# aleflabo/MoCoDAD

Hardware: AMD Instinct MI355X
Metric: pose-clips/sec (whole node) @ noise_steps=10, 5 seeds; AUC vs ref (higher is better)
Workload: dtype f32

## Files before the change

### mocodad_amd/csrc/mcd_device.hpp

```cpp

#pragma once
#include <hip/hip_runtime.h>
#include <stdint.h>
#include <string.h>
#include <stdlib.h>
#include <math.h>
#include <string>
#include <vector>
#include <unordered_map>
#include <utility>
#include <type_traits>
#include <atomic>

#include "../../include/mocodad_hip.h"
#include "mcd_chain.hpp"

namespace mcd {

typedef float f32x4 __attribute__((ext_vector_type(4)));
typedef float f32x2 __attribute__((ext_vector_type(2)));
typedef const float __attribute__((address_space(4))) cfloat;
typedef const float __attribute__((address_space(1))) gfloat;
typedef const f32x4 __attribute__((address_space(1))) gf32x4;
__device__ __forceinline__ gfloat* as_global(const float* p) { return (gfloat*)p; }
typedef float __attribute__((address_space(3))) lds_float;
typedef f32x4 __attribute__((address_space(3))) lds_f32x4;
__device__ __forceinline__ unsigned lds_addr(const float* p) { return (unsigned)(uintptr_t)p; }
__device__ __forceinline__ float4 lds_load4(unsigned addr) {
    const f32x4 v = *(lds_f32x4*)(uintptr_t)addr;
    return make_float4(v[0], v[1], v[2], v[3]);
}
__device__ __forceinline__ void lds_store4(unsigned addr, float a, float b, float c, float d) {
    *(lds_f32x4*)(uintptr_t)addr = f32x4{a, b, c, d};
}
typedef f32x4 __attribute__((address_space(1))) gf32x4_rw;
__device__ __forceinline__ void store_global4(float* p, float4 v) {
    *(gf32x4_rw*)p = f32x4{v.x, v.y, v.z, v.w};
}
__device__ __forceinline__ float4 load_global4(const float* p) {
    const f32x4 v = *(gf32x4*)p;
    return make_float4(v[0], v[1], v[2], v[3]);
}

#ifndef MCD_NWAVES
#define MCD_NWAVES 8
#endif
constexpr int NWAVES = MCD_NWAVES;
constexpr int NTHREADS = NWAVES * 64;
constexpr int EDIM = 16;
constexpr int NLAYERS = 11;
constexpr int EMB_TOTAL = 532;
constexpr int EMB_STRIDE = 536;

__host__ __device__ constexpr int cs_of(int c) { return c + 4; }
__host__ __device__ constexpr int ceil16(int x) { return (x + 15) / 16 * 16; }

struct LDesc { int cin, cout, V, res; };
__host__ __device__ constexpr LDesc layer_desc(int l) {
    return l == 0 ? LDesc{16, 16, 17, 1}  : l == 1 ? LDesc{16, 32, 17, 1} : l == 2 ? LDesc{32, 32, 17, 0}
         : l == 3 ? LDesc{32, 64, 12, 1} : l == 4 ? LDesc{64, 64, 12, 0} : l == 5 ? LDesc{64, 128, 10, 1}
         : l == 6 ? LDesc{128, 64, 10, 1} : l == 7 ? LDesc{64, 64, 12, 0} : l == 8 ? LDesc{64, 32, 12, 1}
         : l == 9 ? LDesc{32, 32, 17, 0} : LDesc{32, 2, 17, 1};
}
__host__ __device__ constexpr int emb_off(int l) {
    return l == 0 ? 0 : l == 1 ? 16 : l == 2 ? 48 : l == 3 ? 80 : l == 4 ? 144 : l == 5 ? 208 : l == 6 ? 336
         : l == 7 ? 400 : l == 8 ? 464 : l == 9 ? 496 : 528;
}

constexpr int TAB_FLOATS = 256;
enum { F_TQ = 0, F_AM = 1, F_WP = 2, F_BIAS = 3, F_SLOPE = 4, F_STRIDE = 8 };
constexpr int TAB_WE = 88, TAB_BE = 89;
constexpr int TAB_RSW = 90, TAB_RSB = 94;
typedef const int __attribute__((address_space(4))) cint;
__device__ __forceinline__ int tab_i(const float* base, int idx) { return ((cint*)base)[idx]; }
__device__ __forceinline__ float tab_f(const float* base, int idx) { return ((cfloat*)base)[idx]; }
template <bool U32>
__device__ __forceinline__ const float* wptr(const float* wb, int off) {
    if constexpr (U32) return reinterpret_cast<const float*>(reinterpret_cast<const char*>(wb) + 4u * (unsigned)off);
    else return wb + off;
}
struct LayerW { int tq, am, wp, bias; float slope; };
__device__ __forceinline__ LayerW layer_w(const float* base, int l) {
    LayerW w;
    w.tq = tab_i(base, l * F_STRIDE + F_TQ); w.am = tab_i(base, l * F_STRIDE + F_AM);
    w.wp = tab_i(base, l * F_STRIDE + F_WP); w.bias = tab_i(base, l * F_STRIDE + F_BIAS);
    w.slope = tab_f(base, l * F_STRIDE + F_SLOPE);
    return w;
}

#ifdef MCD_PROFILE
constexpr int PROF_STAGE = 72;
constexpr int PROF_BAR = 30;
constexpr int PROF_NW = NWAVES;
constexpr int PROF_SLOTS = PROF_STAGE + PROF_NW + PROF_BAR * PROF_NW;
constexpr int PROF_TRACE = 128;
#endif
struct Prof {
#ifdef MCD_PROFILE
    unsigned* acc;
    unsigned long long tlast;
    bool on;
    bool won;
    int bidx;
    int wv;
    unsigned* tr;
    bool tr_on;
    __device__ __forceinline__ void trace(int slot) {
        if (tr_on) tr[slot * PROF_NW + wv] = (unsigned)__builtin_readcyclecounter();
    }
    __device__ __forceinline__ void mark(int id) {
        if (on) {
            const unsigned long long t = __builtin_readcyclecounter();
            __hip_atomic_fetch_add(acc + id, (unsigned)(t - tlast), __ATOMIC_RELAXED, __HIP_MEMORY_SCOPE_WORKGROUP);
            tlast = t;
        }
    }
    __device__ __forceinline__ void sync() {
        const unsigned long long t0 = __builtin_readcyclecounter();
        __syncthreads();
        const unsigned long long t1 = __builtin_readcyclecounter();
        if (won && bidx < PROF_BAR)
            __hip_atomic_fetch_add(acc + PROF_STAGE + PROF_NW + bidx * PROF_NW + wv, (unsigned)(t1 - t0), __ATOMIC_RELAXED, __HIP_MEMORY_SCOPE_WORKGROUP);
        ++bidx;
    }
    __device__ __forceinline__ void off() { on = false; won = false; acc = nullptr; tlast = 0; bidx = 0; wv = 0; tr = nullptr; tr_on = false; }
#else
    __device__ __forceinline__ void trace(int) {}
    __device__ __forceinline__ void mark(int) {}
    __device__ __forceinline__ void sync() { __syncthreads(); }
    __device__ __forceinline__ void off() {}
#endif
};
#define bsync() prof.sync()
#define STAGE(id) prof.mark(id)

__device__ __forceinline__ float prelu_bound(float a) {
    return __int_as_float(__float_as_int(a) <= 0x3f800000 ? 0x7f800000 : (int)0xff800000);
}
__device__ __forceinline__ float prelu(float x, float a) { return __builtin_amdgcn_fmed3f(x, a * x, prelu_bound(a)); }

template <int CTRL>
__device__ __forceinline__ float dpp_f(float v) {
    return __int_as_float(__builtin_amdgcn_update_dpp(0, __float_as_int(v), CTRL, 0xf, 0xf, true));
}
__device__ __forceinline__ float row16_sum(float v) {
    v += dpp_f<0xB1>(v);
    v += dpp_f<0x4E>(v);
    v += dpp_f<0x141>(v);
    v += dpp_f<0x140>(v);
    return v;
}

template <int L, bool PAD = false>
__device__ __forceinline__ void fmac_bc(float& acc, float coef, float y) {
    if (PAD)
        asm("v_fmac_f32_dpp %0, %1, %2 row_newbcast:%3 row_mask:0xf bank_mask:0xf\n\ts_nop 1" : "+v"(acc) : "v"(coef), "v"(y), "n"(L));
    else
        asm("v_fmac_f32_dpp %0, %1, %2 row_newbcast:%3 row_mask:0xf bank_mask:0xf" : "+v"(acc) : "v"(coef), "v"(y), "n"(L));
}
template <int L, bool PAD = false>
__device__ __forceinline__ float mul_bc(float coef, float y) {
    float r;
    if (PAD)
        asm("v_mul_f32_dpp %0, %1, %2 row_newbcast:%3 row_mask:0xf bank_mask:0xf\n\ts_nop 1" : "=v"(r) : "v"(coef), "v"(y), "n"(L));
    else
        asm("v_mul_f32_dpp %0, %1, %2 row_newbcast:%3 row_mask:0xf bank_mask:0xf" : "=v"(r) : "v"(coef), "v"(y), "n"(L));
    return r;
}
#define MCD_DPP(OP, I) OP " %[y" #I "], %[c" #I "], %[x] row_newbcast:%[L] row_mask:0xf bank_mask:0xf\n\t"
#define MCD_TM_IN(I) [c##I] "v"(c[I])
#define MCD_TM2(OP, CON, NOP) asm(MCD_DPP(OP, 0) MCD_DPP(OP, 1) NOP : [y0] CON(y[0]), [y1] CON(y[1]) \
                                  : MCD_TM_IN(0), MCD_TM_IN(1), [x] "v"(x), [L] "n"(L))
#define MCD_TM3(OP, CON, NOP) asm(MCD_DPP(OP, 0) MCD_DPP(OP, 1) MCD_DPP(OP, 2) NOP : [y0] CON(y[0]), [y1] CON(y[1]), [y2] CON(y[2]) \
                                  : MCD_TM_IN(0), MCD_TM_IN(1), MCD_TM_IN(2), [x] "v"(x), [L] "n"(L))
#define MCD_TM4(OP, CON, NOP) asm(MCD_DPP(OP, 0) MCD_DPP(OP, 1) MCD_DPP(OP, 2) MCD_DPP(OP, 3) NOP \
                                  : [y0] CON(y[0]), [y1] CON(y[1]), [y2] CON(y[2]), [y3] CON(y[3]) \
                                  : MCD_TM_IN(0), MCD_TM_IN(1), MCD_TM_IN(2), MCD_TM_IN(3), [x] "v"(x), [L] "n"(L))
#define MCD_TM5(OP, CON, NOP) asm(MCD_DPP(OP, 0) MCD_DPP(OP, 1) MCD_DPP(OP, 2) MCD_DPP(OP, 3) MCD_DPP(OP, 4) NOP \
                                  : [y0] CON(y[0]), [y1] CON(y[1]), [y2] CON(y[2]), [y3] CON(y[3]), [y4] CON(y[4]) \
                                  : MCD_TM_IN(0), MCD_TM_IN(1), MCD_TM_IN(2), MCD_TM_IN(3), MCD_TM_IN(4), [x] "v"(x), [L] "n"(L))
#define MCD_TM6(OP, CON, NOP) asm(MCD_DPP(OP, 0) MCD_DPP(OP, 1) MCD_DPP(OP, 2) MCD_DPP(OP, 3) MCD_DPP(OP, 4) MCD_DPP(OP, 5) NOP \
                                  : [y0] CON(y[0]), [y1] CON(y[1]), [y2] CON(y[2]), [y3] CON(y[3]), [y4] CON(y[4]), [y5] CON(y[5]) \
                                  : MCD_TM_IN(0), MCD_TM_IN(1), MCD_TM_IN(2), MCD_TM_IN(3), MCD_TM_IN(4), MCD_TM_IN(5), [x] "v"(x), [L] "n"(L))
#define MCD_TM(N) do { if constexpr (INIT) { if constexpr (PAD) MCD_TM##N("v_mul_f32_dpp", "=&v", "s_nop 1"); else MCD_TM##N("v_mul_f32_dpp", "=&v", ""); } \
                       else { if constexpr (PAD) MCD_TM##N("v_fmac_f32_dpp", "+v", "s_nop 1"); else MCD_TM##N("v_fmac_f32_dpp", "+v", ""); } } while (0)
template <int QC, int L, bool INIT, bool PAD>
__device__ __forceinline__ void tm_step(float (&y)[QC], const float (&c)[QC], float x) {
    static_assert(QC >= 1 && QC <= 6, "time-mix group sizes");
    if constexpr (QC == 1) {
        if constexpr (INIT) y[0] = mul_bc<L, PAD>(c[0], x);
        else fmac_bc<L, PAD>(y[0], c[0], x);
    } else if constexpr (QC == 2) {
        MCD_TM(2);
    } else if constexpr (QC == 3) {
        MCD_TM(3);
    } else if constexpr (QC == 4) {
        MCD_TM(4);
    } else if constexpr (QC == 5) {
        MCD_TM(5);
    } else {
        MCD_TM(6);
    }
}
template <int... Is, class F>
__device__ __forceinline__ void static_for_impl(std::integer_sequence<int, Is...>, F&& f) {
    (f(std::integral_constant<int, Is>{}), ...);
}
template <int N, class F>
__device__ __forceinline__ void static_for(F&& f) { static_for_impl(std::make_integer_sequence<int, N>{}, f); }

constexpr int MIX_QPAD = 4;

__host__ __device__ constexpr int mix_vmap(int V, int ks, int g) {
    return ks < 2 * (((V + 3) / 4) / 2) ? 8 * (ks >> 1) + 2 * (ks & 1) + 4 * (g & 1) + (g >> 1) : 8 * (((V + 3) / 4) / 2) + g;
}

template <int CIN, int V, int T, int NB>
struct MixCfg {
    static constexpr int KS = (V + 3) / 4;
    static constexpr int KP = 2 * (KS / 2);
    static constexpr int MT = (V + 15) / 16;
    static constexpr int CB = CIN / 16;
    static constexpr int QALL = (T % 3 == 0) ? 3 : (T % 2 == 0) ? 2 : T == 5 ? 3 : (T == 7 || T == 11) ? 4 : 1;
    static constexpr int Q2 = (T % 2 == 0 || T == 5 || T == 7 || T == 11) ? 2 : 1;
    static constexpr int units_of(int qc) { return NB * CB * ((T + qc - 1) / qc); }
    static constexpr int Q6 = (T == 12) ? 6 : 1;
    static constexpr int Q5 = (T == 10) ? 5 : 1, Q4 = (T == 8) ? 4 : 1;
    static constexpr int measured_qc() {
        if (NB == 1 && NWAVES == 12 && T >= 7) return CIN >= 64 ? (T == 10 && CIN == 64 ? 5 : T >= 10 ? 4 : 3) : CIN == 32 ? 2 : 1;
        if (NB != 1 || NWAVES != 8) return 0;
        if (CIN == 32 && (T == 5 || T == 9 || T == 10 || T == 11)) return 3;
        if (CIN == 16 && T == 9) return 2;
        return 0;
    }
    static constexpr int QX = measured_qc();
    static constexpr int QC = QX > 0 ? QX : (Q6 > 1 && units_of(Q6) >= NWAVES) ? Q6 : (Q5 > 1 && units_of(Q5) >= NWAVES) ? Q5
                            : (Q4 > 1 && units_of(Q4) >= NWAVES) ? Q4 : units_of(QALL) >= NWAVES ? QALL : units_of(Q2) >= NWAVES ? Q2
                            : 2 * units_of(QALL) > NWAVES ? QALL : 2 * units_of(Q2) > NWAVES ? Q2 : 1;
    static constexpr int NQ = (T + QC - 1) / QC;
    static constexpr bool RAGGED = NQ * QC != T;
    static_assert(NQ * QC - T < MIX_QPAD, "zero rows behind the coefficient tables");
    static constexpr int UNITS = NB * CB * NQ;
    static constexpr int PER = (UNITS + NWAVES - 1) / NWAVES;
    static constexpr int NR = (KS * T + 15) / 16;
    static constexpr bool SAMEQ = NQ == 3 && UNITS == 12 && NWAVES == 8;
    static_assert(T > 12 || PER == 1 || UNITS % NWAVES == 0 || SAMEQ, "mix units: a partial round of units (see MixCfg::QX)");
    __device__ static __forceinline__ int unit_of(int wave, int round) {
        if constexpr (SAMEQ) {
            if (wave < 4) return (wave >> 1) + NQ * ((wave & 1) * 2 + round);
            return round == 0 ? 2 + NQ * (wave - 4) : -1;
        } else {
            const int u = wave + round * NWAVES;
            return u < UNITS ? u : -1;
        }
    }
};
template <int CIN, int V, int T, int NB>
struct MixCoef {
    using M = MixCfg<CIN, V, T, NB>;
    float tq[M::QC][M::NR], aop[M::QC][M::MT][M::KS];
    __device__ __forceinline__ void load(const float* tqd, const float* af, int wave, int lane) {
        load_unit(tqd, af, M::unit_of(wave, 0), lane);
    }
    __device__ __forceinline__ void load_unit(const float* tqd, const float* af, int u, int lane) {
        gfloat* tqd_g = as_global(tqd);
        gfloat* af_g = as_global(af);
        const int uc = u < 0 ? 0 : (u < M::UNITS ? u : M::UNITS - 1);
        const int q0 = (uc % M::NQ) * M::QC;
#pragma unroll
        for (int qi = 0; qi < M::QC; ++qi) {
#pragma unroll
            for (int r = 0; r < M::NR; ++r) tq[qi][r] = tqd_g[((q0 + qi) * M::NR + r) * 64 + lane];
#pragma unroll
            for (int mt = 0; mt < M::MT; ++mt)
#pragma unroll
                for (int ks = 0; ks < M::KS; ++ks) aop[qi][mt][ks] = af_g[(((q0 + qi) * M::MT + mt) * M::KS + ks) * 64 + lane];
        }
    }
};

struct ChIdx {
    int cb16, j;
    __device__ __forceinline__ operator int() const { return cb16 + j; }
};
struct ZeroInit { __device__ __forceinline__ float operator()(int, int, int, int) const { return 0.f; } };
template <int CIN, int V, int T, int NB, bool FORCE = false, bool SCORE = false, class Init, class Store>
__device__ __forceinline__ void mix_stage(const float* __restrict__ in, int cs_in, const MixCoef<CIN, V, T, NB>& pre,
                                          const float* __restrict__ tqd, const float* __restrict__ af, int wave, int lane,
                                          Init&& init, Store&& store) {
    using M = MixCfg<CIN, V, T, NB>;
    constexpr int KS = M::KS, KP = M::KP, MT = M::MT, CB = M::CB, QC = M::QC, NQ = M::NQ, PER = M::PER;
    constexpr bool XB32 = FORCE || SCORE;
    const int j = lane & 15, g = lane >> 4;
    const int voff_pair = 4 * (g & 1) + (g >> 1);
    auto load_x = [&](int u, float (&x)[KS][T]) {
        const int rest = u / NQ;
        const int cb = rest % CB, n = rest / CB;
        unsigned ua = lds_addr(in) + 4u * (unsigned)(n * (T * V) * cs_in + cb * 16);
        asm volatile("" : "+s"(ua));
        const lds_float* ub = (const lds_float*)(uintptr_t)ua;
        const lds_float* a_p = ub + (__mul24(voff_pair, cs_in) + j);
        const lds_float* a_l = (V == 17) ? ub + j : ub + (__mul24(g, cs_in) + j);
        static_for<KS>([&](auto si) {
            constexpr int ks = decltype(si)::value;
            constexpr int vbase = ks < KP ? 8 * (ks >> 1) + 2 * (ks & 1) : 4 * KP;
            const lds_float* xb = ks < KP ? a_p : a_l;
#pragma unroll
            for (int t = 0; t < T; ++t) {
                if constexpr (XB32) x[ks][t] = ((const volatile lds_float*)xb)[(t * V + vbase) * cs_in];
                else x[ks][t] = xb[(t * V + vbase) * cs_in];
            }
        });
    };
    auto unit = [&](const MixCoef<CIN, V, T, NB>& cur, int u, const float (&xs)[KS][T]) {
        const int q0 = (u % NQ) * QC, rest = u / NQ;
        const int cb = rest % CB, n = rest / CB;
        constexpr bool J16 = V == 17;
        constexpr int MTM = J16 ? 1 : MT;
        constexpr bool ZINIT = std::is_same_v<std::decay_t<Init>, ZeroInit>;
        static_assert(ZINIT || !J16, "a seeded accumulator (W-first layers) on a 17-joint layer: joint 16's seed is not wired up");
        f32x4 acc[QC][MTM];
        float part[QC];
#pragma unroll
        for (int qi = 0; qi < QC; ++qi) {
            part[qi] = 0.f;
#pragma unroll
            for (int mt = 0; mt < MTM; ++mt)
                if ((M::RAGGED && q0 + qi >= T) || ZINIT) {
                    acc[qi][mt] = f32x4{0.f, 0.f, 0.f, 0.f};
                } else {
                    acc[qi][mt] = init(n, q0 + qi, mt * 16 + j, ChIdx{cb * 16, 4 * g});
                }
        }
        static_for<KS>([&](auto si) {
            constexpr int ks = decltype(si)::value;
            const float (&x)[T] = xs[ks];
            float y[QC];
            static_for<T>([&](auto ti) {
                constexpr int t = decltype(ti)::value;
                float c[QC];
#pragma unroll
                for (int qi = 0; qi < QC; ++qi) c[qi] = cur.tq[qi][(ks * T + t) / 16];
                tm_step<QC, (ks * T + t) % 16, t == 0, t == T - 1>(y, c, x[t]);
            });
            static_for<QC>([&](auto qq) {
                constexpr int qi = decltype(qq)::value;
#pragma unroll
                for (int mt = 0; mt < MTM; ++mt)
                    acc[qi][mt] = __builtin_amdgcn_mfma_f32_16x16x4f32(y[qi], cur.aop[qi][mt][ks], acc[qi][mt], 0, 0, 0);
                if constexpr (J16) part[qi] = fmaf(cur.aop[qi][1][ks], y[qi], part[qi]);
            });
        });
#pragma unroll
        for (int qi = 0; qi < QC; ++qi) {
            if (M::RAGGED && q0 + qi >= T) continue;
#pragma unroll
            for (int mt = 0; mt < MTM; ++mt) {
                if ((mt + 1) * 16 <= V || mt * 16 + j < V) store(n, q0 + qi, mt * 16 + j, ChIdx{cb * 16, 4 * g}, acc[qi][mt]);
            }
            if constexpr (J16) {
                const unsigned u = __float_as_uint(part[qi]);
                const auto h = __builtin_amdgcn_permlane32_swap(u, u, false, false);
                const unsigned v2 = __float_as_uint(__uint_as_float(h[0]) + __uint_as_float(h[1]));
                const auto f = __builtin_amdgcn_permlane16_swap(v2, v2, false, false);
                const float z16 = __uint_as_float(f[0]) + __uint_as_float(f[1]);
                if (g == 0) store(n, q0 + qi, 16, ChIdx{cb * 16, j}, z16);
            }
        }
    };
    {
        MixCoef<CIN, V, T, NB> cur = pre;
        static_for<PER>([&](auto ri) {
            constexpr int rnd = decltype(ri)::value;
            constexpr bool ALLW = (FORCE || SCORE) && !M::SAMEQ && M::UNITS == PER * NWAVES;
            const int u = ALLW ? wave + rnd * NWAVES : M::unit_of(wave, rnd);
            constexpr bool SURE = ALLW;
            float xs[KS][T];
            load_x(SURE ? u : (u < 0 ? 0 : u), xs);
            if constexpr (FORCE) __builtin_amdgcn_sched_barrier(0);
            MixCoef<CIN, V, T, NB> nxt;
            if constexpr (rnd + 1 < PER && !M::SAMEQ && NQ > 1) nxt.load_unit(tqd, af, M::unit_of(wave, rnd + 1), lane);
            if (SURE || u >= 0) unit(cur, u, xs);
            if constexpr (rnd + 1 < PER && !M::SAMEQ && NQ > 1) cur = nxt;
        });
    }
}
template <int CIN, int V, int T, int NB, class Init, class Store>
__device__ __forceinline__ void mix_stage(const float* __restrict__ in, int cs_in, const float* __restrict__ tqd,
                                          const float* __restrict__ af, int wave, int lane, Init&& init, Store&& store) {
    MixCoef<CIN, V, T, NB> mc;
    mc.load(tqd, af, wave, lane);
    mix_stage<CIN, V, T, NB>(in, cs_in, mc, tqd, af, wave, lane, init, store);
}

template <int C, int VIN, int VOUT, int T, int NB, bool CAPTURE>
struct RsCfg {
    static constexpr int KS = CAPTURE ? (VIN > 16 ? 5 : 4) : (VIN + 3) / 4;
    static constexpr int MT = (VOUT + 15) / 16;
    static constexpr int CB = C / 16;
    static constexpr int UNITS = NB * T * CB;
    static constexpr int PER = (UNITS + NWAVES - 1) / NWAVES;
    static constexpr int VS = CAPTURE ? VIN : VOUT;
    static constexpr int SK = VS > 16 ? 5 : 4;
    static constexpr bool ALIGNED = NB * CB == NWAVES && PER == T;
};
__host__ __device__ constexpr int rs_vmap(bool capture, int vin, int ks, int g) {
    return capture ? (ks < 4 ? 4 * g + ks : 16 + g) : mix_vmap(vin, ks, g);
}

template <int C, int VIN, int VOUT, int T, int NB, bool CAPTURE>
struct RsCoef {
    using RC = RsCfg<C, VIN, VOUT, T, NB, CAPTURE>;
    float aop[RC::MT][RC::KS];
    float bias[RC::MT][4];
    __device__ __forceinline__ void load(const float* wf, const float* bdp, int lane) {
        gfloat* wf_g = as_global(wf);
        gfloat* bdp_g = as_global(bdp);
        const int g = lane >> 4;
#pragma unroll
        for (int mt = 0; mt < RC::MT; ++mt)
#pragma unroll
            for (int ks = 0; ks < RC::KS; ++ks) aop[mt][ks] = wf_g[(mt * RC::KS + ks) * 64 + lane];
#pragma unroll
        for (int mt = 0; mt < RC::MT; ++mt)
#pragma unroll
            for (int r = 0; r < 4; ++r) bias[mt][r] = bdp_g[mt * 16 + 4 * g + r];
    }
};

template <int C, int VIN, int VOUT, int T, int NB, bool CAPTURE, bool ADD, bool ILP = false, bool SQMAP = false, int NSK>
__device__ __forceinline__ void resample_stage(const float* __restrict__ in, int cs_in, float* __restrict__ out, int cs_out,
                                               const RsCoef<C, VIN, VOUT, T, NB, CAPTURE>& rc,
                                               float (&skip)[NSK], int wave, int lane) {
    using RC = RsCfg<C, VIN, VOUT, T, NB, CAPTURE>;
    constexpr int KS = RC::KS, MT = RC::MT, CB = RC::CB, UNITS = RC::UNITS, PER = RC::PER, SK = RC::SK;
    static_assert(!(CAPTURE || ADD) || NSK == PER * SK, "skip register count");
    constexpr int KP = 2 * (((VIN + 3) / 4) / 2);
    const int j = lane & 15, g = lane >> 4;
    const auto& aop = rc.aop;
    const auto& bias = rc.bias;
    float xr[CAPTURE ? 1 : PER][CAPTURE ? 1 : KS] = {};
    constexpr bool FULL = (CAPTURE || ADD) && UNITS == PER * NWAVES;
    using SM = std::conditional_t<SQMAP, MixCfg<(SQMAP ? C : 32), (SQMAP ? (CAPTURE ? VOUT : VIN) : 12), (SQMAP ? T : 3), (SQMAP ? NB : 2)>, MixCfg<32, 12, 3, 2>>;
    static_assert(!SQMAP || (SM::SAMEQ && UNITS == SM::UNITS && PER == SM::PER && !RC::ALIGNED), "SQMAP: the 12-unit SAMEQ mixes only");
    auto unit_at = [&](int i, int& cb, int& nt) -> bool {
        if constexpr (SQMAP) {
            const int um = SM::unit_of(wave, i);
            const int uu = um < 0 ? 0 : um, grp = uu / SM::NQ;
            cb = grp % CB; nt = (grp / CB) * T + uu % SM::NQ;
            return um >= 0;
        } else {
            const int u = wave + i * NWAVES;
            cb = RC::ALIGNED ? wave % CB : u % CB; nt = RC::ALIGNED ? (wave / CB) * T + i : u / CB;
            return FULL || u < UNITS;
        }
    };
    static_for<PER>([&](auto pi) {
        constexpr int i = decltype(pi)::value;
        int cb, nt;
        if (unit_at(i, cb, nt)) {
            const float* ub = in + (nt * VIN * cs_in + cb * 16);
            const float* a_main = ub + (__mul24(CAPTURE ? 4 * g : 4 * (g & 1) + (g >> 1), cs_in) + j);
            const float* a_tail = CAPTURE ? ub + j : ub + (__mul24(g, cs_in) + j);
            static_for<KS>([&](auto si) {
                constexpr int ks = decltype(si)::value;
                constexpr bool MAIN = CAPTURE ? ks < 4 : ks < KP;
                constexpr int row0 = CAPTURE ? (ks < 4 ? ks : 16) : (ks < KP ? 8 * (ks >> 1) + 2 * (ks & 1) : 4 * KP);
                const float xv = (MAIN ? a_main : a_tail)[row0 * cs_in];
                if constexpr (CAPTURE) skip[i * SK + ks] = xv;
                else xr[i][ks] = xv;
            });
        }
    });
    constexpr bool J16 = VOUT == 17;
    constexpr int MTM = J16 ? 1 : MT;
    auto finish = [&](auto pi, f32x4 (&acc)[MTM], float part) {
        constexpr int i = decltype(pi)::value;
        int cb, nt;
        unit_at(i, cb, nt);
        if constexpr (ADD) {
#pragma unroll
            for (int r = 0; r < 4; ++r) acc[0][r] += skip[i * SK + r];
            if constexpr (SK == 5 && !J16) acc[MT - 1][0] += skip[i * SK + 4];
        }
        float* uo = out + (nt * VOUT * cs_out + cb * 16);
        float* zo = uo + (__mul24(4 * g, cs_out) + j);
#pragma unroll
        for (int mt = 0; mt < MTM; ++mt)
#pragma unroll
            for (int r = 0; r < 4; ++r)
                if (mt * 16 + 4 * g + r < VOUT) zo[(mt * 16 + r) * cs_out] = acc[mt][r];
        if constexpr (J16) {
            const unsigned pu = __float_as_uint(part);
            const auto h = __builtin_amdgcn_permlane32_swap(pu, pu, false, false);
            const unsigned v2 = __float_as_uint(__uint_as_float(h[0]) + __uint_as_float(h[1]));
            const auto f = __builtin_amdgcn_permlane16_swap(v2, v2, false, false);
            float z16 = __uint_as_float(f[0]) + __uint_as_float(f[1]) + bias[1][0];
            if constexpr (ADD && SK == 5) z16 += skip[i * SK + 4];
            if (g == 0) uo[16 * cs_out + j] = z16;
        }
    };
    if constexpr (ILP) {
        f32x4 acc[PER][MTM];
        float part[PER];
#pragma unroll
        for (int i = 0; i < PER; ++i) {
            part[i] = 0.f;
#pragma unroll
            for (int mt = 0; mt < MTM; ++mt) acc[i][mt] = f32x4{bias[mt][0], bias[mt][1], bias[mt][2], bias[mt][3]};
        }
        static_for<KS>([&](auto si) {
            constexpr int ks = decltype(si)::value;
            static_for<PER>([&](auto pi) {
                constexpr int i = decltype(pi)::value;
                float x;
                if constexpr (CAPTURE) x = skip[i * SK + ks]; else x = xr[i][ks];
#pragma unroll
                for (int mt = 0; mt < MTM; ++mt) acc[i][mt] = __builtin_amdgcn_mfma_f32_16x16x4f32(aop[mt][ks], x, acc[i][mt], 0, 0, 0);
                if constexpr (J16) part[i] = fmaf(aop[1][ks], x, part[i]);
            });
        });
        static_for<PER>([&](auto pi) {
            int cb_, nt_;
            if (unit_at(decltype(pi)::value, cb_, nt_)) finish(pi, acc[decltype(pi)::value], part[decltype(pi)::value]);
        });
    } else {
        static_for<PER>([&](auto pi) {
            constexpr int i = decltype(pi)::value;
            int cb_, nt_;
            if (unit_at(i, cb_, nt_)) {
                f32x4 acc[MTM];
                float part = 0.f;
#pragma unroll
                for (int mt = 0; mt < MTM; ++mt) acc[mt] = f32x4{bias[mt][0], bias[mt][1], bias[mt][2], bias[mt][3]};
                static_for<KS>([&](auto si) {
                    constexpr int ks = decltype(si)::value;
                    float x;
                    if constexpr (CAPTURE) x = skip[i * SK + ks]; else x = xr[i][ks];
#pragma unroll
                    for (int mt = 0; mt < MTM; ++mt) acc[mt] = __builtin_amdgcn_mfma_f32_16x16x4f32(aop[mt][ks], x, acc[mt], 0, 0, 0);
                    if constexpr (J16) part = fmaf(aop[1][ks], x, part);
                });
                finish(pi, acc, part);
            }
        });
    }
}

__host__ __device__ constexpr int cmax(int a, int b) { return a > b ? a : b; }

template <int MT, int NT>
struct Tiling {
    static constexpr int MW = MT > NWAVES ? MT / NWAVES : 1;
    static constexpr int NG = MT > NWAVES ? 1 : NWAVES / MT;
    static constexpr int MAXN = (NT + NG - 1) / NG;
};
template <int MT, int KQ>
__device__ __forceinline__ void load_afrags(const float4* __restrict__ wp, int wave, int lane, float4 (&a)[KQ], int mi = 0) {
    const float* wpl = reinterpret_cast<const float*>(wp + (((wave + mi * NWAVES) % MT) * KQ) * 64 + lane);
#pragma unroll
    for (int kq = 0; kq < KQ; ++kq) a[kq] = load_global4(wpl + kq * 256);
}

struct NoPre { static constexpr bool none = true; };
template <int MT, int NT, int KQ1, int KQ2, bool IDRES, bool FORCE = false, bool DUAL = FORCE, bool SLOTK = false, class Epi, class Pre = NoPre>
__device__ __forceinline__ void gemm_tiles(const float4 (&a)[KQ1 + KQ2], const float* __restrict__ b1, int cs1,
                                           const float* __restrict__ b2, int cs2, int wave, int lane, Epi&& epi, int mi = 0,
                                           const float4 cinit = make_float4(0.f, 0.f, 0.f, 0.f), Pre&& pre = Pre{}) {
    constexpr bool HASPRE = !std::is_same_v<std::decay_t<Pre>, NoPre>;
    constexpr int NG = Tiling<MT, NT>::NG;
    constexpr int MAXN = Tiling<MT, NT>::MAXN;
    const int mt = (wave + mi * NWAVES) % MT, ng = MT > NWAVES ? 0 : wave / MT;
    if (NWAVES % MT != 0 && MT <= NWAVES && ng >= NG) return;
    const int j = lane & 15, g = lane >> 4;
    const int c0 = mt * 16 + 4 * g;
    const int col0 = ng * 16 + j;
    const float* const p1b = b1 + __mul24(col0, cs1) + 4 * g;
    const float* const p2b = b2 + __mul24(col0, cs2) + 4 * g;
    constexpr int KQ = KQ1 + KQ2;
    constexpr int DEPTH0 = KQ < 3 ? KQ : 3;
    auto one_tile = [&](auto ii) {
        constexpr int i = decltype(ii)::value;
        const int col = col0 + i * NG * 16;
        f32x4 c = {cinit.x, cinit.y, cinit.z, cinit.w};
        const float* p1 = p1b + i * NG * 16 * cs1;
        const float* p2 = p2b + i * NG * 16 * cs2;
        if (IDRES) {
            const float4 r = *reinterpret_cast<const float4*>(p2 - 4 * g + c0);
            c[0] = r.x; c[1] = r.y; c[2] = r.z; c[3] = r.w;
        }
        auto rd = [&](auto kk) {
            constexpr int kq = decltype(kk)::value;
            return *reinterpret_cast<const float4*>(kq < KQ1 ? p1 + kq * 16 : p2 + (kq - KQ1) * 16);
        };
        float4 buf[DEPTH0];
        static_for<DEPTH0>([&](auto dd) { buf[decltype(dd)::value] = rd(dd); });
        float4 pe = make_float4(0.f, 0.f, 0.f, 0.f);
        if constexpr (HASPRE) pe = pre(ii, col, ng);
        if constexpr (FORCE) __builtin_amdgcn_sched_barrier(0);
        static_for<KQ>([&](auto kk) {
            constexpr int kq = decltype(kk)::value;
            const float4 u = buf[kq % DEPTH0];
            if constexpr (kq + DEPTH0 < KQ) buf[kq % DEPTH0] = rd(std::integral_constant<int, kq + DEPTH0>{});
            if constexpr (FORCE) __builtin_amdgcn_sched_barrier(0);
            c = __builtin_amdgcn_mfma_f32_16x16x4f32(a[kq].x, u.x, c, 0, 0, 0);
            c = __builtin_amdgcn_mfma_f32_16x16x4f32(a[kq].y, u.y, c, 0, 0, 0);
            c = __builtin_amdgcn_mfma_f32_16x16x4f32(a[kq].z, u.z, c, 0, 0, 0);
            c = __builtin_amdgcn_mfma_f32_16x16x4f32(a[kq].w, u.w, c, 0, 0, 0);
        });
        if constexpr (HASPRE) epi(ii, col, c0, c, col0, ng, pe);
        else epi(ii, col, c0, c, col0, ng);
    };
    auto two_tiles = [&](auto ia, auto ib) {
        constexpr int i0 = decltype(ia)::value, i1 = decltype(ib)::value;
        const float* p1[2] = {p1b + i0 * NG * 16 * cs1, p1b + i1 * NG * 16 * cs1};
        const float* p2[2] = {p2b + i0 * NG * 16 * cs2, p2b + i1 * NG * 16 * cs2};
        f32x4 c[2];
#pragma unroll
        for (int h = 0; h < 2; ++h) {
            c[h] = f32x4{cinit.x, cinit.y, cinit.z, cinit.w};
            if (IDRES) {
                const float4 r = *reinterpret_cast<const float4*>(p2[h] - 4 * g + c0);
                c[h][0] = r.x; c[h][1] = r.y; c[h][2] = r.z; c[h][3] = r.w;
            }
        }
        auto rd = [&](int h, auto kk) {
            constexpr int kq = decltype(kk)::value;
            return *reinterpret_cast<const float4*>(kq < KQ1 ? p1[h] + kq * 16 : p2[h] + (kq - KQ1) * 16);
        };
        float4 buf[2][DEPTH0];
        static_for<DEPTH0>([&](auto dd) { buf[0][decltype(dd)::value] = rd(0, dd); buf[1][decltype(dd)::value] = rd(1, dd); });
        float4 pe0 = make_float4(0.f, 0.f, 0.f, 0.f), pe1 = pe0;
        if constexpr (HASPRE) { pe0 = pre(ia, col0 + i0 * NG * 16, ng); pe1 = pre(ib, col0 + i1 * NG * 16, ng); }
        __builtin_amdgcn_sched_barrier(0);
        static_for<KQ>([&](auto kk) {
            constexpr int kq = decltype(kk)::value;
            const float4 u0 = buf[0][kq % DEPTH0], u1 = buf[1][kq % DEPTH0];
            if constexpr (kq + DEPTH0 < KQ) {
                buf[0][kq % DEPTH0] = rd(0, std::integral_constant<int, kq + DEPTH0>{});
                buf[1][kq % DEPTH0] = rd(1, std::integral_constant<int, kq + DEPTH0>{});
            }
            __builtin_amdgcn_sched_barrier(0);
            c[0] = __builtin_amdgcn_mfma_f32_16x16x4f32(a[kq].x, u0.x, c[0], 0, 0, 0);
            c[1] = __builtin_amdgcn_mfma_f32_16x16x4f32(a[kq].x, u1.x, c[1], 0, 0, 0);
            c[0] = __builtin_amdgcn_mfma_f32_16x16x4f32(a[kq].y, u0.y, c[0], 0, 0, 0);
            c[1] = __builtin_amdgcn_mfma_f32_16x16x4f32(a[kq].y, u1.y, c[1], 0, 0, 0);
            c[0] = __builtin_amdgcn_mfma_f32_16x16x4f32(a[kq].z, u0.z, c[0], 0, 0, 0);
            c[1] = __builtin_amdgcn_mfma_f32_16x16x4f32(a[kq].z, u1.z, c[1], 0, 0, 0);
            c[0] = __builtin_amdgcn_mfma_f32_16x16x4f32(a[kq].w, u0.w, c[0], 0, 0, 0);
            c[1] = __builtin_amdgcn_mfma_f32_16x16x4f32(a[kq].w, u1.w, c[1], 0, 0, 0);
        });
        if constexpr (HASPRE) {
            epi(ia, col0 + i0 * NG * 16, c0, c[0], col0, ng, pe0);
            epi(ib, col0 + i1 * NG * 16, c0, c[1], col0, ng, pe1);
        } else {
            epi(ia, col0 + i0 * NG * 16, c0, c[0], col0, ng);
            epi(ib, col0 + i1 * NG * 16, c0, c[1], col0, ng);
        }
    };
    constexpr bool PIPE = DUAL && MAXN >= 2 && !HASPRE;
    constexpr int PW = DUAL ? 2 : 1;
    constexpr int DEPTH = PIPE ? 1 : DEPTH0;
    if constexpr (PIPE) {
        constexpr int NP = (MAXN + PW - 1) / PW;
        const int nv = (NT - ng + NG - 1) / NG;
        float4 bufs[2][2][DEPTH];
        float4 seed[2][2];
        f32x4 accs[2][2];
        auto rdt = [&](int i, auto kk) {
            constexpr int kq = decltype(kk)::value;
            return *reinterpret_cast<const float4*>(kq < KQ1 ? p1b + i * NG * 16 * cs1 + kq * 16 : p2b + i * NG * 16 * cs2 + (kq - KQ1) * 16);
        };
        auto fetch = [&](auto pp, auto dd) {
            constexpr int p = decltype(pp)::value, d = decltype(dd)::value;
            if constexpr (p < NP) {
                constexpr int i0 = PW * p, i1 = (PW == 2 && i0 + 1 < MAXN) ? i0 + 1 : i0;
                bufs[p & 1][0][d] = rdt(i0, dd);
                if constexpr (i1 != i0) bufs[p & 1][1][d] = rdt(i1, dd);
                if constexpr (IDRES && d == DEPTH - 1 && NWAVES == 12) {
                    seed[p & 1][0] = *reinterpret_cast<const float4*>(p2b + i0 * NG * 16 * cs2 - 4 * g + c0);
                    if constexpr (i1 != i0) seed[p & 1][1] = *reinterpret_cast<const float4*>(p2b + i1 * NG * 16 * cs2 - 4 * g + c0);
                }
            }
        };
        auto epi_pair = [&](auto pp, auto nn) {
            constexpr int p = decltype(pp)::value, N = decltype(nn)::value, i0 = PW * p, i1 = i0 + 1;
            epi(std::integral_constant<int, i0>{}, col0 + i0 * NG * 16, c0, accs[p & 1][0], col0, ng);
            if constexpr (N == 2) epi(std::integral_constant<int, i1>{}, col0 + i1 * NG * 16, c0, accs[p & 1][1], col0, ng);
        };
        auto chain = [&](auto pp, auto nn) {
            constexpr int p = decltype(pp)::value, N = decltype(nn)::value, i0 = PW * p, i1 = N == 2 ? i0 + 1 : i0;
            f32x4 (&c)[2] = accs[p & 1];
#pragma unroll
            for (int h = 0; h < N; ++h) {
                c[h] = f32x4{cinit.x, cinit.y, cinit.z, cinit.w};
                if (IDRES) {
                    if constexpr (NWAVES != 12) seed[p & 1][h] = *reinterpret_cast<const float4*>(p2b + (h ? i1 : i0) * NG * 16 * cs2 - 4 * g + c0);
                    c[h] = f32x4{seed[p & 1][h].x, seed[p & 1][h].y, seed[p & 1][h].z, seed[p & 1][h].w};
                }
            }
            static_for<KQ>([&](auto kk) {
                constexpr int kq = decltype(kk)::value;
                float4 u[2];
#pragma unroll
                for (int h = 0; h < N; ++h) u[h] = bufs[p & 1][h][kq % DEPTH];
                if constexpr (kq + DEPTH < KQ) {
                    bufs[p & 1][0][kq % DEPTH] = rdt(i0, std::integral_constant<int, kq + DEPTH>{});
                    if constexpr (N == 2) bufs[p & 1][1][kq % DEPTH] = rdt(i1, std::integral_constant<int, kq + DEPTH>{});
                } else if constexpr (N == PW) {
                    fetch(std::integral_constant<int, p + 1>{}, std::integral_constant<int, kq + DEPTH - KQ>{});
                }
                __builtin_amdgcn_sched_barrier(0);
                c[0] = __builtin_amdgcn_mfma_f32_16x16x4f32(a[kq].x, u[0].x, c[0], 0, 0, 0);
                if constexpr (N == 2) c[1] = __builtin_amdgcn_mfma_f32_16x16x4f32(a[kq].x, u[1].x, c[1], 0, 0, 0);
                c[0] = __builtin_amdgcn_mfma_f32_16x16x4f32(a[kq].y, u[0].y, c[0], 0, 0, 0);
                if constexpr (N == 2) c[1] = __builtin_amdgcn_mfma_f32_16x16x4f32(a[kq].y, u[1].y, c[1], 0, 0, 0);
                c[0] = __builtin_amdgcn_mfma_f32_16x16x4f32(a[kq].z, u[0].z, c[0], 0, 0, 0);
                if constexpr (N == 2) c[1] = __builtin_amdgcn_mfma_f32_16x16x4f32(a[kq].z, u[1].z, c[1], 0, 0, 0);
                c[0] = __builtin_amdgcn_mfma_f32_16x16x4f32(a[kq].w, u[0].w, c[0], 0, 0, 0);
                if constexpr (N == 2) c[1] = __builtin_amdgcn_mfma_f32_16x16x4f32(a[kq].w, u[1].w, c[1], 0, 0, 0);
                if constexpr (kq == 0 && p > 0) {
                    __builtin_amdgcn_sched_barrier(0);
                    epi_pair(std::integral_constant<int, p - 1>{}, std::integral_constant<int, PW>{});
                    __builtin_amdgcn_sched_barrier(0);
                }
            });
            if (PW * (p + 1) >= nv) epi_pair(pp, nn);
        };
        static_for<DEPTH>([&](auto dd) { fetch(std::integral_constant<int, 0>{}, dd); });
        static_for<NP>([&](auto pp) {
            constexpr int i0 = PW * decltype(pp)::value, i1 = i0 + 1;
            if constexpr (PW == 2 && i1 < MAXN) {
                if (i1 < nv) chain(pp, std::integral_constant<int, 2>{});
                else if (i0 < nv) chain(pp, std::integral_constant<int, 1>{});
            } else {
                if (i0 < nv) chain(pp, std::integral_constant<int, 1>{});
            }
        });
    } else if constexpr (DUAL && MAXN >= 2) {
        static_for<(MAXN + 1) / 2>([&](auto pp) {
            constexpr int i0 = 2 * decltype(pp)::value, i1 = i0 + 1;
            if constexpr (i1 < MAXN) {
                if (ng + i1 * NG < NT) two_tiles(std::integral_constant<int, i0>{}, std::integral_constant<int, i1>{});
                else if (ng + i0 * NG < NT) one_tile(std::integral_constant<int, i0>{});
            } else {
                if (ng + i0 * NG < NT) one_tile(std::integral_constant<int, i0>{});
            }
        });
    } else {
        static_for<MAXN>([&](auto ii) {
            if constexpr (SLOTK && (decltype(ii)::value + 1) * NG <= NT) one_tile(ii);
            else if (ng + decltype(ii)::value * NG < NT) one_tile(ii);
        });
    }
}

struct NoHook { __device__ __forceinline__ void operator()() const {} };

template <int KQ>
struct LayerAfr {
    float4 a[KQ];
    float4 bcur;
    template <int MT, bool U32 = false>
    __device__ __forceinline__ void load(const float* wb, const LayerW& lw, int wave, int lane) {
        load_afrags<MT, KQ>(reinterpret_cast<const float4*>(wptr<U32>(wb, lw.wp)), wave, lane, a);
        bcur = load_global4(wptr<U32>(wb, lw.bias) + (wave % MT) * 16 + 4 * (lane >> 4));
    }
};

template <int CIN, int COUT, int V, bool RES, bool HASEMB, int T, int NB, bool FORCE = false, int CSX = cs_of(CIN), bool SLOTSEL = false, class H1, class H2>
__device__ __forceinline__ void layer_generic(const float* wb, const LayerW lw, const MixCoef<CIN, V, T, NB>& mc,
                                              const float* __restrict__ in, float* __restrict__ z, float* __restrict__ out,
                                              const float* __restrict__ embl, int wave, int lane, Prof& prof, int prof_id,
                                              H1&& pre_gemm, H2&& pre_barrier,
                                              const LayerAfr<(CIN / 16) * (RES ? 2 : 1)>* pre_afr = nullptr) {
    constexpr int MT = ceil16(COUT) / 16;
    constexpr int COLS = NB * T * V;
    constexpr int NT = ceil16(COLS) / 16;
    constexpr int TV = T * V;
    constexpr int CSI = cs_of(CIN), CSO = cs_of(COUT);
    constexpr int KQ1 = CIN / 16, KQ2 = RES ? CIN / 16 : 0;
    float4 afr[KQ1 + KQ2];
    const int trs = 8 + 8 * ((prof_id - 32) / 3);
    prof.trace(trs + 0);
    constexpr bool TSEL = SLOTSEL && HASEMB && NB == 2 && T == 3;
    const float* bias = wptr<TSEL>(wb, lw.bias);
    float4 bcur;
    if (pre_afr != nullptr) {
#pragma unroll
        for (int k = 0; k < KQ1 + KQ2; ++k) afr[k] = pre_afr->a[k];
        bcur = pre_afr->bcur;
    } else {
        load_afrags<MT, KQ1 + KQ2>(reinterpret_cast<const float4*>(wptr<TSEL>(wb, lw.wp)), wave, lane, afr);
        bcur = load_global4(bias + (wave % MT) * 16 + 4 * (lane >> 4));
    }
    mix_stage<CIN, V, T, NB, FORCE, HASEMB>(in, CSX, mc, wptr<TSEL>(wb, lw.tq), wptr<TSEL>(wb, lw.am), wave, lane,
                             ZeroInit{},
                             [&](int n, int q, int w, ChIdx c, auto v) {
                                 float* zp = (z + (n * (T * V) * CSI + q * (V * CSI) + c.cb16)) + (__mul24(w, CSI) + c.j);
                                 if constexpr (std::is_same_v<decltype(v), f32x4>) lds_store4(lds_addr(zp), v[0], v[1], v[2], v[3]);
                                 else *zp = v;
                             });
    prof.trace(trs + 1);
    pre_gemm();
    bsync();
    prof.trace(trs + 2);
    prof.mark(prof_id);
    const float slope = lw.slope;
    const float pinf = prelu_bound(slope);
    constexpr int TILE_STEP = Tiling<MT, NT>::NG * 16;
    constexpr bool FOLD = RES;
    unsigned oaddr = 0, eaddr = 0;
    auto set_bases = [&](int mi) {
        const int mt = (wave + mi * NWAVES) % MT, ng = MT > NWAVES ? 0 : wave / MT;
        const int c0 = mt * 16 + 4 * (lane >> 4);
        oaddr = lds_addr(out) + 4u * (unsigned)(__mul24(ng * 16 + (lane & 15), CSO) + c0);
        eaddr = HASEMB ? lds_addr(embl) + 4u * (unsigned)c0 : 0u;
        asm volatile("" : "+v"(oaddr), "+v"(eaddr));
    };
    set_bases(0);
    constexpr bool EHOIST = HASEMB && NB == 1 && FORCE;
    float4 e_pre = make_float4(0.f, 0.f, 0.f, 0.f);
    if constexpr (EHOIST) e_pre = lds_load4(eaddr);
    auto emb_of = [&](auto ti, int col, int ng) -> float4 {
        if constexpr (TSEL) {
            constexpr int I = decltype(ti)::value, NG = Tiling<MT, NT>::NG;
            constexpr int t_lo = I * NG, t_hi = t_lo + NG - 1 < NT - 1 ? t_lo + NG - 1 : NT - 1;
            constexpr int t_st = TV % 16 != 0 ? TV / 16 : -1;
            constexpr unsigned HI = 4u * EMB_STRIDE;
            if constexpr ((t_hi + 1) * 16 <= TV) {
                return lds_load4(eaddr);
            } else if constexpr (t_lo * 16 >= TV) {
                return lds_load4(eaddr + HI);
            } else if constexpr (t_st < t_lo || t_st > t_hi) {
                return lds_load4(eaddr + ((ng + t_lo) * 16 >= TV ? HI : 0u));
            } else {
                unsigned a = eaddr + (t_st == t_hi ? 0u : t_st == t_lo ? HI : ng > t_st - t_lo ? HI : 0u);
                if (ng == t_st - t_lo) {
                    a = eaddr + (col >= TV ? HI : 0u);
                    asm volatile("" : "+v"(a));
                }
                return lds_load4(a);
            }
        } else if constexpr (NB == 2) {
            const int tile_lo = (ng + decltype(ti)::value * Tiling<MT, NT>::NG) * 16;
            unsigned eo = tile_lo >= TV ? 4u * EMB_STRIDE : 0u;
            if (tile_lo < TV && tile_lo + 16 > TV) {
                eo = col >= TV ? 4u * EMB_STRIDE : 0u;
                asm volatile("" : "+v"(eo));
            }
            return lds_load4(eaddr + eo);
        } else if constexpr (NB > 2) {
            const int n = col / TV;
            return lds_load4(eaddr + 4u * (unsigned)((n < NB ? n : NB - 1) * EMB_STRIDE));
        } else if constexpr (EHOIST) {
            return e_pre;
        } else {
            return lds_load4(eaddr);
        }
    };
    constexpr bool EPRE = HASEMB && NB > 1 && FORCE;
    auto epi = [&](auto ti, int col, int c0, f32x4 acc, int, int ng, auto... pe) {
        if (COUT % 16 == 0 || c0 < COUT) {
            float4 e = make_float4(0.f, 0.f, 0.f, 0.f);
            if constexpr (sizeof...(pe) > 0) e = (pe, ...);
            else if constexpr (HASEMB) e = emb_of(ti, col, ng);
            f32x2 t0 = f32x2{acc[0], acc[1]}, t1 = f32x2{acc[2], acc[3]};
            if constexpr (!FOLD) { t0 += f32x2{bcur.x, bcur.y}; t1 += f32x2{bcur.z, bcur.w}; }
            const f32x2 m0 = t0 * slope, m1 = t1 * slope;
            const f32x2 r0 = f32x2{__builtin_amdgcn_fmed3f(t0[0], m0[0], pinf), __builtin_amdgcn_fmed3f(t0[1], m0[1], pinf)} + f32x2{e.x, e.y};
            const f32x2 r1 = f32x2{__builtin_amdgcn_fmed3f(t1[0], m1[0], pinf), __builtin_amdgcn_fmed3f(t1[1], m1[1], pinf)} + f32x2{e.z, e.w};
            constexpr unsigned tile_bytes = 4u * decltype(ti)::value * TILE_STEP * CSO;
            lds_store4(oaddr + tile_bytes, r0[0], r0[1], r1[0], r1[1]);
        }
    };
    prof.trace(trs + 3);
    if constexpr (EPRE) gemm_tiles<MT, NT, KQ1, KQ2, !RES, FORCE, FORCE, TSEL>(afr, z, CSI, in, CSX, wave, lane, epi, 0, FOLD ? bcur : make_float4(0.f, 0.f, 0.f, 0.f), emb_of);
    else gemm_tiles<MT, NT, KQ1, KQ2, !RES, FORCE, FORCE, TSEL>(afr, z, CSI, in, CSX, wave, lane, epi, 0, FOLD ? bcur : make_float4(0.f, 0.f, 0.f, 0.f));
#pragma unroll
    for (int mi = 1; mi < Tiling<MT, NT>::MW; ++mi) {
        load_afrags<MT, KQ1 + KQ2>(reinterpret_cast<const float4*>(wptr<TSEL>(wb, lw.wp)), wave, lane, afr, mi);
        bcur = load_global4(bias + ((wave + mi * NWAVES) % MT) * 16 + 4 * (lane >> 4));
        set_bases(mi);
        if constexpr (EHOIST) e_pre = lds_load4(eaddr);
        if constexpr (EPRE) gemm_tiles<MT, NT, KQ1, KQ2, !RES, FORCE, FORCE, TSEL>(afr, z, CSI, in, CSX, wave, lane, epi, mi, FOLD ? bcur : make_float4(0.f, 0.f, 0.f, 0.f), emb_of);
        else gemm_tiles<MT, NT, KQ1, KQ2, !RES, FORCE, FORCE, TSEL>(afr, z, CSI, in, CSX, wave, lane, epi, mi, FOLD ? bcur : make_float4(0.f, 0.f, 0.f, 0.f));
    }
    prof.trace(trs + 4);
    pre_barrier();
#ifdef MCD_PROFILE
    asm volatile("s_waitcnt lgkmcnt(0)" ::: "memory");
#endif
    prof.trace(trs + 5);
    bsync();
    prof.trace(trs + 6);
    prof.mark(prof_id + 1);
}
template <int CIN, int COUT, int V, bool RES, bool HASEMB, int T, int NB>
__device__ __forceinline__ void layer_generic(const float* wb, const LayerW lw, const float* __restrict__ in,
                                              float* __restrict__ z, float* __restrict__ out,
                                              const float* __restrict__ embl, int wave, int lane, Prof& prof, int prof_id) {
    MixCoef<CIN, V, T, NB> mc;
    mc.load(wb + lw.tq, wb + lw.am, wave, lane);
    layer_generic<CIN, COUT, V, RES, HASEMB, T, NB>(wb, lw, mc, in, z, out, embl, wave, lane, prof, prof_id, NoHook{}, NoHook{});
}

template <int L, int T, int NB>
using LMix = MixCoef<layer_desc(L).cin, layer_desc(L).V, T, NB>;
template <int L>
using LAfr = LayerAfr<(layer_desc(L).cin / 16) * (layer_desc(L).res ? 2 : 1)>;
template <int L, bool U32 = false>
__device__ __forceinline__ void load_lafr(LAfr<L>& A, const float* wb, int wave, int lane) {
    A.template load<ceil16(layer_desc(L).cout) / 16, U32>(wb, layer_w(wb, L), wave, lane);
}
template <int L, int T, int NB, bool FORCE = false, int CSX = cs_of(layer_desc(L).cin), class H1, class H2>
__device__ __forceinline__ void layer_std(const float* wb, const LMix<L, T, NB>& mc, const float* in, float* z, float* out,
                                          const float* emb, int wave, int lane, Prof& prof, H1&& pre_gemm, H2&& pre_barrier,
                                          const LAfr<L>* pre_afr = nullptr) {
    constexpr LDesc D = layer_desc(L);
    layer_generic<D.cin, D.cout, D.V, D.res != 0, true, T, NB, FORCE, CSX, true>(wb, layer_w(wb, L), mc, in, z, out, emb + emb_off(L), wave, lane,
                                                               prof, 32 + 3 * L, pre_gemm, pre_barrier, pre_afr);
}

struct EmbRow {
    float4 w[4];
    float b;
    template <bool U32 = false>
    __device__ __forceinline__ void load(const float* wb, int o) {
        const float* we = wptr<U32>(wb, tab_i(wb, TAB_WE));
#pragma unroll
        for (int q = 0; q < 4; ++q) w[q] = load_global4(we + o * EDIM + 4 * q);
        b = as_global(wptr<U32>(wb, tab_i(wb, TAB_BE)))[o];
    }
};
template <int NB>
__device__ __forceinline__ void emb_row(const EmbRow& f, int o, const float* __restrict__ se, float* __restrict__ emb,
                                        float* __restrict__ e10) {
#pragma unroll
    for (int n = 0; n < NB; ++n) {
        f32x2 acc = {f.b, 0.f};
#pragma unroll
        for (int q = 0; q < 4; ++q) {
            const float4 sv = *reinterpret_cast<const float4*>(se + n * EDIM + 4 * q);
            acc = f32x2{f.w[q].x, f.w[q].y} * f32x2{sv.x, sv.y} + acc;
            acc = f32x2{f.w[q].z, f.w[q].w} * f32x2{sv.z, sv.w} + acc;
        }
        const float r = acc[0] + acc[1];
        if (o < emb_off(10)) emb[n * EMB_STRIDE + o] = r;
        else if (o < EMB_TOTAL) e10[n * 4 + (o - emb_off(10))] = r;
    }
}
constexpr int EMB_EXTRA = EMB_TOTAL > NTHREADS ? EMB_TOTAL - NTHREADS : 0;
template <int NB>
__device__ __forceinline__ void emb_compute(const EmbRow& f, const float* __restrict__ exw, const float* __restrict__ se,
                                            float* __restrict__ emb, float* __restrict__ e10, int tid) {
    static_assert(EMB_TOTAL <= 2 * NTHREADS, "two rows per thread cover the embedding outputs");
    emb_row<NB>(f, tid, se, emb, e10);
    if (tid < EMB_EXTRA) {
        EmbRow f2;
#pragma unroll
        for (int q = 0; q < 4; ++q) f2.w[q] = *reinterpret_cast<const float4*>(exw + tid * 20 + 4 * q);
        f2.b = exw[tid * 20 + 16];
        emb_row<NB>(f2, tid + NTHREADS, se, emb, e10);
    }
}

template <int T, int NB>
struct Plan {
    static constexpr int NBT = NB * T;
    static constexpr int P17 = ceil16(NBT * 17), P12 = ceil16(NBT * 12), P10 = ceil16(NBT * 10);
    static constexpr int s16 = P17 * 20, s32a = P17 * 36, s32b = P12 * 36, s64b = P12 * 68, s64c = P10 * 68, s128 = P10 * 132;
    static constexpr int L0_in = 0, L0_z = s16, L0_out = 2 * s16;
    static constexpr int L1_in = 2 * s16, L1_z = 0, L1_out = 3 * s16;
    static constexpr int L2_in = 3 * s16, L2_z = 0, L2_out = 3 * s16 + s32a;
    static constexpr int DN1_out = 0;
    static constexpr int L3_in = 0, L3_z = s32b, L3_out = 2 * s32b;
    static constexpr int L4_in = 2 * s32b, L4_z = 2 * s32b + s64b, L4_out = 0;
    static constexpr int DN2_out = s128 + s64c;
    static constexpr int L5_in = s128 + s64c, L5_z = s128, L5_out = 0;
    static constexpr int L6_in = 0, L6_p = s128;
    static constexpr int UP3_out = 0;
    static constexpr int L7_in = 0, L7_z = s64b, L7_out = 2 * s64b;
    static constexpr int L8_in = 2 * s64b, L8_z = 0, L8_out = s64b;
    static constexpr int L8_p = 0;
    static constexpr int UP2_out = cmax(s64b + s32b, 2 * s32a);
    static constexpr int L9_in = UP2_out, L9_z = 0, L9_out = s32a;
    static constexpr int L10_in = s32a, L10_p = 2 * s32a;
    static constexpr int R = cmax(cmax(cmax(s128 + 2 * s64c, 2 * s128), cmax(3 * s16 + 2 * s32a, 2 * s32b + 2 * s64b)),
                                  cmax(cmax(3 * s64b, 3 * s32a), UP2_out + s32a));
    static_assert(s32a <= 3 * s16 && s64b <= 2 * s32b && s32a <= s64b && s64b <= s128, "LDS plan: regions would overlap");
    static constexpr int XT = P17 * 4;
    static constexpr int EMB = NB * EMB_STRIDE;
    static constexpr int EAUX = 2 * 4 * 4 + 4 * EDIM;
    static constexpr int ZN = P17 * 2;
    static constexpr int WM = 12;
    static constexpr int BIA = 64 + 16 + 32;
    static constexpr int UPD = 16;
    static constexpr int ZO = P17 * 2;
    static constexpr int TT = P17 * 2;
    static constexpr int CE = 4 * EDIM;
    static constexpr int LOSS = NB * 64;
    static constexpr int EXW = EMB_EXTRA * 20;
#ifdef MCD_PROFILE
    static constexpr int PROFTR = (NB * T >= 10 && NWAVES <= 12) ? PROF_TRACE * PROF_NW : 0;
    static constexpr int PROF = PROF_SLOTS + PROFTR;
#else
    static constexpr int PROF = 0;
#endif
    static constexpr int TOTAL = R + XT + EMB + EAUX + ZN + WM + BIA + UPD + ZO + TT + CE + LOSS + EXW + PROF;
    static_assert((size_t)TOTAL * 4 <= 160 * 1024, "LDS plan: more than 160 KB");
    static constexpr size_t BYTES = (size_t)TOTAL * 4;
};

}
```

### mocodad_amd/csrc/mcd_score_kernel.hpp

```cpp
#pragma once
#include "mcd_device.hpp"
#include "mcd_encode_kernel.hpp"

namespace mcd {

template <int T, int NB, int MINW, bool LT = false>
__global__ __launch_bounds__(NTHREADS, MINW) void score_kernel(const ScoreParams P) {
    using PL = Plan<T, NB>;
    constexpr int TV17 = T * 17;
    constexpr int COLS17 = NB * TV17;
    extern __shared__ __attribute__((aligned(16))) float smem[];
    float* const RG = smem;
    float* const XT = RG + PL::R;
    float* const EMB = XT + PL::XT;
    float* const E10 = EMB + PL::EMB;
    float* const SEN = E10 + 32;
    float* const ZN = E10 + PL::EAUX;
    int* const WM = reinterpret_cast<int*>(ZN + PL::ZN);
    float* const BIA = reinterpret_cast<float*>(WM + PL::WM);
    int* const UPD = reinterpret_cast<int*>(BIA + PL::BIA);
    float* const ZO = reinterpret_cast<float*>(UPD + PL::UPD);

    const int tid0 = threadIdx.x;
    int tid = tid0;
    int lane = tid & 63;
    int wave = __builtin_amdgcn_readfirstlane(tid >> 6);
    Prof prof;
    prof.off();
#ifdef MCD_PROFILE
    const unsigned long long wg_t0 = __builtin_amdgcn_s_memrealtime();
#endif
    if (P.phase > 0 && blockIdx.x * 2 >= gridDim.x) {
        const unsigned long long t0 = __builtin_readcyclecounter();
        while (__builtin_readcyclecounter() - t0 < (unsigned long long)P.phase * 1024ull) __builtin_amdgcn_s_sleep(32);
    }
    if (P.phase < -15) {
        const unsigned h = (blockIdx.x * 2654435761u) >> 26;
        const unsigned long long t0 = __builtin_readcyclecounter();
        while (__builtin_readcyclecounter() - t0 < (unsigned long long)h * (unsigned long long)(-P.phase) * 16ull) __builtin_amdgcn_s_sleep(32);
    }
    const int grp = blockIdx.x / P.split, part = blockIdx.x - grp * P.split;
    const int win0 = grp * NB;
    const int Tx = P.n_corrupt;
    auto window_of = [&](int n) { const int b = win0 + n; return b < P.B ? b : P.B - 1; };
    if (threadIdx.x < NB) {
        const int b = window_of(threadIdx.x);
        WM[threadIdx.x] = P.win_mask ? P.win_mask[b] : (int)P.fixed_mask;
        WM[4 + threadIdx.x] = b;
        if (threadIdx.x == 0) { WM[8] = 0; WM[9] = -1; }
    }
    if (threadIdx.x >= 128 && threadIdx.x < 128 + NB * T) {
        const int i = threadIdx.x - 128, n = i / T, t = i % T;
        const int fixed = P.win_mask ? P.win_mask[window_of(n)] : (int)P.fixed_mask;
        const int k = P.win_mask ? (((fixed >> t) & 1) ? -1 : 0) : P.upd_of[t];
        UPD[i] = k < 0 ? -1 : (n * T + (P.win_mask ? t : P.pos_of[k])) * 17;
    }
    static_assert(NB <= 4 && T <= 16 && NB * T <= 16, "tail index packing: 4 bits (chain, frame) | 2 bits chain | 4 bits frame");
    int* const TT = reinterpret_cast<int*>(ZO + PL::ZO);
    float* const CE = reinterpret_cast<float*>(TT + PL::TT);
    float* const LOSSB = CE + PL::CE;
    float* const EXW = LOSSB + PL::LOSS;
    if constexpr (MINW >= 4) {
        if (threadIdx.x == 0) {
            int sh = P.prio_shift;
            if (sh > 0 && P.tune) {
                const int sig = (int)gridDim.x * 1009 + P.S * 31 + P.ns;
                const int ticks = P.tune[1];
                if (P.tune[0] == sig && ticks > 0) {
                    const unsigned v = (unsigned)(((unsigned long long)(unsigned)ticks * (unsigned)(P.prio_rounds > 0 ? P.prio_rounds : 1)) / 6u) | 1u;
                    sh = 31 - __clz((int)v);
                    if ((v >> (sh > 0 ? sh - 1 : 0)) & 1u) ++sh;
                    sh = sh < 10 ? 10 : (sh > 26 ? 26 : sh);
                }
            }
            UPD[15] = sh;
            UPD[14] = (int)(unsigned)__builtin_amdgcn_s_memrealtime();
        }
    }
    for (int u = threadIdx.x; u < EMB_EXTRA * 17; u += NTHREADS) {
        const int r = u / 17, k = u % 17;
        EXW[r * 20 + k] = k < 16 ? P.wbuf[tab_i(P.wbuf, TAB_WE) + (NTHREADS + r) * EDIM + k] : P.wbuf[tab_i(P.wbuf, TAB_BE) + NTHREADS + r];
    }
    for (int u = threadIdx.x; u < COLS17 * C0; u += NTHREADS) {
        const int col = u / C0, n = col / TV17, t = (col / 17) % T, v = col % 17;
        TT[u] = (n * T + t) | (n << 4) | (t << 6) | (v << 10);
    }
    if (threadIdx.x < 64) BIA[threadIdx.x] = P.wbuf[tab_i(P.wbuf, 6 * F_STRIDE + F_BIAS) + threadIdx.x];
    else if (threadIdx.x < 64 + C0) BIA[threadIdx.x] = P.wbuf[tab_i(P.wbuf, 10 * F_STRIDE + F_BIAS) + threadIdx.x - 64];
    else if (threadIdx.x >= 80 && threadIdx.x < 112) BIA[threadIdx.x] = P.wbuf[tab_i(P.wbuf, 8 * F_STRIDE + F_BIAS) + threadIdx.x - 80];
    const int CTV = C0 * Tx * 17;
    const int K = P.ns > 2 ? P.ns - 1 : 1;

    if (P.cond_inkernel) {
        static_assert(CondFastLds<T, NB>::FLOATS <= PL::R, "cond_fast_body's region does not fit the work region zeroed for it");
        int enc_solo = -1;
        do {
            for (int u = tid; u < PL::R; u += NTHREADS) smem[u] = 0.f;
            bsync();
            cond_fast_body<T, NB, (NB > 1)>(P.wbuf, P.dv, [&](int t) { return P.cond_idx[t]; }, P.seg_len, smem, win0, P.B, CE, nullptr, enc_solo);
            bsync();
            if constexpr (NB == 1) break;
            enc_solo = next_nonfinite_slot<NB>(CE, enc_solo, win0, P.B);
        } while (enc_solo >= 0);
    } else if (threadIdx.x < NB * EDIM) {
        CE[threadIdx.x] = P.cond_emb ? P.cond_emb[(size_t)window_of(threadIdx.x / EDIM) * EDIM + threadIdx.x % EDIM] : 0.f;
    }
    for (int u = tid; u < PL::R + PL::XT; u += NTHREADS) smem[u] = 0.f;
    bsync();

#ifdef MCD_PROFILE
    prof.acc = reinterpret_cast<unsigned*>(EXW + PL::EXW);
    for (int i = tid0; i < PROF_SLOTS; i += NTHREADS) prof.acc[i] = 0u;
    prof.on = (tid0 == 0 && blockIdx.x == 0 && P.prof != nullptr); prof.tlast = __builtin_readcyclecounter();
    prof.won = ((tid0 & 63) == 0 && blockIdx.x == 0 && P.prof != nullptr); prof.wv = tid0 >> 6;
    prof.tr = (P.prof && PL::PROFTR) ? prof.acc + PROF_SLOTS : nullptr;
    for (int i = tid0; i < PL::PROFTR; i += NTHREADS) prof.acc[PROF_SLOTS + i] = 0u;
    __syncthreads();
#endif
    auto lt_inject = [&](int id, float* region, int cs, int C, int V) {
        if constexpr (LT) {
            if (P.lt_stage == id) {
                bsync();
                for (int u = threadIdx.x; u < NB * C * T * V; u += NTHREADS) {
                    const int v = u % V, t = (u / V) % T, c = (u / (V * T)) % C, n = u / (V * T * C);
                    const int b = window_of(n);
                    region[((n * T + t) * V + v) * cs + c] = P.lt_in[(((size_t)b * C + c) * T + t) * V + v];
                }
                bsync();
            }
        }
    };
    auto lt_dump = [&](int id, const float* region, int cs, int C, int V) {
        if constexpr (LT) {
            if (P.lt_stage == id) {
                bsync();
                for (int u = threadIdx.x; u < NB * C * T * V; u += NTHREADS) {
                    const int v = u % V, t = (u / V) % T, c = (u / (V * T)) % C, n = u / (V * T * C);
                    const int b = win0 + n;
                    if (b < P.B) P.lt_out[(((size_t)b * C + c) * T + t) * V + v] = region[((n * T + t) * V + v) * cs + c];
                }
                bsync();
            }
        }
    };
    using RS1 = RsCfg<32, 17, 12, T, NB, true>;
    using RS2 = RsCfg<64, 12, 10, T, NB, true>;
    float skip1[RS1::PER * RS1::SK];
    float skip2[RS2::PER * RS2::SK];
    constexpr bool LOWO = MINW <= (NWAVES == 12 ? 3 : 2);
    constexpr bool TSEL = T == 3 && NB == 2;

    const int i_first = P.mode == 1 ? P.step_single : P.ns - 1;
    const int i_last = P.mode == 1 ? P.step_single : 1;
    auto silu_row = [&](int step, int t_id) {
        if (t_id >= 0 && t_id < NB * EDIM) {
            const int solo = NB > 1 ? WM[9] : -1;
            const float e = P.step_table[step * (4 + EDIM) + 4 + (t_id % EDIM)] + ((solo >= 0 && t_id / EDIM != solo) ? 0.f : CE[t_id]);
            SEN[t_id] = e / (1.f + expf(-e));
        }
    };
    for (int s = part; s < P.S; s += P.split) {
    typedef const ScoreParams __attribute__((address_space(4))) KScoreParams;
    KScoreParams* Q = (KScoreParams*)__builtin_amdgcn_kernarg_segment_ptr();
    asm volatile("" : "+s"(Q));
    int tid_s = tid0;
    asm volatile("" : "+v"(tid_s));
    {
        DataView dv;
        dv.data = Q->dv.data; dv.base = Q->dv.base; dv.sc = Q->dv.sc; dv.st = Q->dv.st; dv.trans = Q->dv.trans; dv.aff = Q->dv.aff;
        const float* noise = Q->noise;
        const float* x_in = Q->x_in;
        const int mode = Q->mode, seg_len = Q->seg_len, Bq = Q->B;
        const unsigned long long seed = Q->seed;
        const long long first_window = Q->first_window;
        for (int u = tid_s; u < COLS17; u += NTHREADS) {
            const int n = u / TV17, t = (u / 17) % T, v = u % 17;
            const int b = WM[4 + n];
            const int fixed = WM[n];
            const int solo = NB > 1 ? WM[9] : -1;
            float xv[C0];
#pragma unroll
            for (int c = 0; c < C0; ++c) {
                if (solo >= 0 && n != solo) {
                    xv[c] = 0.f;
                } else if (mode == 1) {
                    xv[c] = x_in ? x_in[((b * C0 + c) * T + t) * 17 + v] : 0.f;
                } else if ((fixed >> t) & 1) {
                    xv[c] = load_coord(dv, b, c, fm_src(P, t), v, seg_len);
                } else {
                    const int e = (c * Tx + fm_tx(P, fixed, t)) * 17 + v;
                    if (noise) xv[c] = noise[((size_t)(s * K + 0) * Bq + b) * CTV + e];
                    else xv[c] = philox_normal(seed, (unsigned)e, 0u, (unsigned)s, (unsigned)(first_window + b));
                }
            }
            XT[u * 4 + 0] = xv[0];
            XT[u * 4 + 1] = xv[1];
        }
    }
    bsync();
    {
        EmbRow er;
        er.load(P.wbuf, tid_s);
        silu_row(i_first, tid_s);
        bsync();
        emb_compute<NB>(er, EXW, SEN, EMB, E10 + (i_first & 1) * 16, tid_s);
        bsync();
    }
    LMix<0, T, NB> mc0;
    mc0.load(P.wbuf + tab_i(P.wbuf, F_TQ), P.wbuf + tab_i(P.wbuf, F_AM), wave, lane);
    constexpr bool WEARLY = T <= 4;
    LAfr<0> A0;
    if constexpr (WEARLY) load_lafr<0>(A0, P.wbuf, wave, lane);
    for (int sidx = i_first; sidx >= i_last; --sidx) {
        const float* srow = P.step_table + sidx * (4 + EDIM);
        const float* wb = P.wbuf;
        asm volatile("" : "+s"(wb));
        tid = tid0;
        asm volatile("" : "+v"(tid));
        lane = tid & 63;
        wave = __builtin_amdgcn_readfirstlane(tid >> 6);
        if constexpr (MINW >= 4) {
            const int sh = UPD[15];
            if (sh > 0) {
                unsigned hwid;
                asm volatile("s_getreg_b32 %0, hwreg(HW_REG_HW_ID)" : "=s"(hwid));
                const unsigned slice = (unsigned)(__builtin_amdgcn_s_memrealtime() >> sh);
                if (((hwid >> 16) ^ slice) & 1u) __builtin_amdgcn_s_setprio(1);
                else __builtin_amdgcn_s_setprio(0);
            }
        }
        constexpr bool NZ_TAIL = MixCfg<16, 17, T, NB>::UNITS <= NWAVES - 2;
        constexpr int NZ_T0 = NZ_TAIL ? NTHREADS - 128 : 0;
        constexpr int NZ_GROUPS = NB * T * 9;
        static_assert(NZ_GROUPS <= 128, "noise groups fit the two idle waves");
        auto noise_part = [&](int t_id) {
            const int gi = t_id - NZ_T0;
            if (P.mode == 0 && sidx > 1 && gi >= 0 && gi < NZ_GROUPS) {
                const int n = gi / (T * 9), r = gi % (T * 9), t = r / 9, v0 = (r % 9) * 2;
                float z[4] = {0.f, 0.f, 0.f, 0.f};
                const int fixed = WM[n];
                const int solo = NB > 1 ? WM[9] : -1;
                if (!((fixed >> t) & 1) && (solo < 0 || n == solo)) {
                    const int b = WM[4 + n];
                    const int tx = fm_tx(P, fixed, t);
                    const int k = P.ns - sidx;
                    if (P.noise) {
                        const float* zp = P.noise + ((size_t)(s * K + k) * P.B + b) * CTV + tx * 17 + v0;
                        z[0] = zp[0]; z[1] = zp[Tx * 17];
                        if (v0 + 1 < 17) { z[2] = zp[1]; z[3] = zp[Tx * 17 + 1]; }
                    } else {
                        philox_normal4(P.seed, (unsigned)(tx * 9 + (v0 >> 1)), (unsigned)k, (unsigned)s, (unsigned)(P.first_window + b), z);
                    }
                }
                float* zo = ZN + ((n * T + t) * 17 + v0) * C0;
                zo[0] = z[0]; zo[1] = z[1];
                if (v0 + 1 < 17) { zo[2] = z[2]; zo[3] = z[3]; }
            }
        };
        noise_part(tid);
        STAGE(0);
        STAGE(1);
#ifdef MCD_PROFILE
        prof.bidx = 0;
        prof.tr_on = prof.won && prof.tr && s == part && sidx == i_first - 1;
        prof.trace(0);
#endif
        auto mixload = [&](auto& mc, int l) { mc.load(wptr<TSEL>(wb, tab_i(wb, l * F_STRIDE + F_TQ)), wptr<TSEL>(wb, tab_i(wb, l * F_STRIDE + F_AM)), wave, lane); };
        auto rsload = [&](auto& rc, int r) { rc.load(wptr<TSEL>(wb, tab_i(wb, TAB_RSW + r)), wptr<TSEL>(wb, tab_i(wb, TAB_RSB + r)), lane); };
        auto mix_early = mixload;
        auto rs_early = rsload;
        NoHook nohook;
        constexpr bool EARLY2 = LOWO || T == 6;
        LMix<1, T, NB> mc1;
        LAfr<1> A1; LAfr<2> A2; LAfr<3> A3; LAfr<4> A4; LAfr<5> A5; LAfr<7> A7; LAfr<9> A9;
        auto wearly = [&](auto& A, auto lc) { if constexpr (WEARLY) load_lafr<decltype(lc)::value, TSEL>(A, wb, wave, lane); };
#define MCD_LC(l) std::integral_constant<int, l>{}
        layer_std<0, T, NB, LOWO, 4>(wb, mc0, XT, RG + PL::L0_z, RG + PL::L0_out, EMB, wave, lane, prof,
                            [&] { mix_early(mc1, 1); }, [&] { wearly(A1, MCD_LC(1)); }, WEARLY ? &A0 : nullptr);
        STAGE(2);
        lt_dump(0, RG + PL::L0_out, 20, 16, 17);
        lt_inject(1, RG + PL::L1_in, 20, 16, 17);
        LMix<2, T, NB> mc2;
        silu_row(sidx > 0 ? sidx - 1 : 0, tid - NZ_T0);
        layer_std<1, T, NB, LOWO>(wb, mc1, RG + PL::L1_in, RG + PL::L1_z, RG + PL::L1_out, EMB, wave, lane, prof,
                            [&] { mix_early(mc2, 2); }, [&] { wearly(A2, MCD_LC(2)); }, WEARLY ? &A1 : nullptr);
        STAGE(3);
        lt_dump(1, RG + PL::L1_out, 36, 32, 17);
        lt_inject(2, RG + PL::L2_in, 36, 32, 17);
        RsCoef<32, 17, 12, T, NB, true> rc1;
        LMix<3, T, NB> mc3;
        layer_std<2, T, NB, LOWO>(wb, mc2, RG + PL::L2_in, RG + PL::L2_z, RG + PL::L2_out, EMB, wave, lane, prof,
                            [&] { rs_early(rc1, 0); }, [&] { if constexpr (EARLY2) mix_early(mc3, 3); }, WEARLY ? &A2 : nullptr);
        STAGE(4);
        lt_dump(2, RG + PL::L2_out, 36, 32, 17);
        lt_inject(11, RG + PL::L2_out, 36, 32, 17);
        if constexpr (!EARLY2) mix_early(mc3, 3);
        constexpr bool SQ12 = !LT && MixCfg<32, 12, T, NB>::SAMEQ;
        resample_stage<32, 17, 12, T, NB, true, false, LOWO, SQ12>(RG + PL::L2_out, 36, RG + PL::DN1_out, 36, rc1, skip1, wave, lane);
        wearly(A3, MCD_LC(3));
        bsync();
        STAGE(5);
        lt_dump(11, RG + PL::DN1_out, 36, 32, 12);
        lt_inject(3, RG + PL::L3_in, 36, 32, 12);
        LMix<4, T, NB> mc4;
        layer_std<3, T, NB, LOWO>(wb, mc3, RG + PL::L3_in, RG + PL::L3_z, RG + PL::L3_out, EMB, wave, lane, prof,
                            [&] { mix_early(mc4, 4); }, [&] { wearly(A4, MCD_LC(4)); }, WEARLY ? &A3 : nullptr);
        STAGE(6);
        lt_dump(3, RG + PL::L3_out, 68, 64, 12);
        lt_inject(4, RG + PL::L4_in, 68, 64, 12);
        RsCoef<64, 12, 10, T, NB, true> rc2;
        LMix<5, T, NB> mc5;
        layer_std<4, T, NB, LOWO>(wb, mc4, RG + PL::L4_in, RG + PL::L4_z, RG + PL::L4_out, EMB, wave, lane, prof,
                            [&] { rs_early(rc2, 1); }, [&] { if constexpr (EARLY2) mix_early(mc5, 5); }, WEARLY ? &A4 : nullptr);
        STAGE(7);
        lt_dump(4, RG + PL::L4_out, 68, 64, 12);
        lt_inject(12, RG + PL::L4_out, 68, 64, 12);
        if constexpr (!EARLY2) mix_early(mc5, 5);
        resample_stage<64, 12, 10, T, NB, true, false, LOWO>(RG + PL::L4_out, 68, RG + PL::DN2_out, 68, rc2, skip2, wave, lane);
        constexpr bool FUSE64 = RS2::ALIGNED && MixCfg<64, 10, T, NB>::QC == T && MixCfg<64, 10, T, NB>::UNITS == NWAVES;
        wearly(A5, MCD_LC(5));
        if constexpr (!FUSE64) bsync();
        STAGE(8);
        lt_dump(12, RG + PL::DN2_out, 68, 64, 10);
        lt_inject(5, RG + PL::L5_in, 68, 64, 10);
        RsCoef<64, 10, 12, T, NB, false> rc3;
        LMix<7, T, NB> mc7;
        {
            constexpr int NT = PL::P10 / 16;
            constexpr int COLS = NB * T * 10;
            const LayerW lw = layer_w(wb, 6);
            float4 afr[8];
            MixCoef<64, 10, T, NB> mc6;
            layer_std<5, T, NB, LOWO>(wb, mc5, RG + PL::L5_in, RG + PL::L5_z, RG + PL::L5_out, EMB, wave, lane, prof, nohook,
                                [&] {
                                    load_afrags<8, 8>(reinterpret_cast<const float4*>(wptr<TSEL>(wb, lw.wp)), wave, lane, afr, 0);
                                    if constexpr (EARLY2) mc6.load(wptr<TSEL>(wb, lw.tq), wptr<TSEL>(wb, lw.am), wave, lane);
                                }, WEARLY ? &A5 : nullptr);
            STAGE(9);
            lt_dump(5, RG + PL::L5_out, 132, 128, 10);
            lt_inject(6, RG + PL::L6_in, 132, 128, 10);
            float* Pb = RG + PL::L6_p;
            if constexpr (!EARLY2) mc6.load(wptr<TSEL>(wb, lw.tq), wptr<TSEL>(wb, lw.am), wave, lane);
            auto epi6 = [&](auto ti, int col, int c0, f32x4 acc, int col0, int) {
                constexpr int STEP = Tiling<8, NT>::NG * 16 * 132;
                constexpr bool FULL = TSEL && (decltype(ti)::value + 1) * Tiling<8, NT>::NG * 16 <= COLS;
                if (FULL || col < COLS) *reinterpret_cast<float4*>(Pb + __mul24(col0, 132) + c0 + decltype(ti)::value * STEP) = make_float4(acc[0], acc[1], acc[2], acc[3]);
            };
            gemm_tiles<8, NT, 8, 0, false, LOWO, LOWO, TSEL>(afr, RG + PL::L6_in, 132, RG + PL::L6_in, 132, wave, lane, epi6, 0);
#pragma unroll
            for (int mi = 1; mi < Tiling<8, NT>::MW; ++mi) {
                load_afrags<8, 8>(reinterpret_cast<const float4*>(wptr<TSEL>(wb, lw.wp)), wave, lane, afr, mi);
                gemm_tiles<8, NT, 8, 0, false, LOWO, LOWO, TSEL>(afr, RG + PL::L6_in, 132, RG + PL::L6_in, 132, wave, lane, epi6, mi);
            }
            if constexpr (EARLY2) { rs_early(rc3, 2); mix_early(mc7, 7); }
            bsync();
            STAGE(10);
            const float slope6 = lw.slope;
            const float pinf6 = prelu_bound(slope6);
            mix_stage<64, 10, T, NB, LOWO, true>(Pb, 132, mc6, wptr<TSEL>(wb, lw.tq), wptr<TSEL>(wb, lw.am), wave, lane,
                                     [&](int n, int q, int w, ChIdx c) {
                                         const float* pp = (Pb + (n * (T * 10) * 132 + q * (10 * 132) + 64 + c.cb16)) + (__mul24(w, 132) + c.j);
                                         const float4 r = lds_load4(lds_addr(pp));
                                         return f32x4{r.x, r.y, r.z, r.w};
                                     },
                                     [&](int n, int q, int w, ChIdx c, f32x4 v) {
                                         const float4 b4 = lds_load4(lds_addr(BIA + c.cb16) + 4u * (unsigned)c.j);
                                         const float4 e4 = lds_load4(lds_addr(EMB + n * EMB_STRIDE + emb_off(6) + c.cb16) + 4u * (unsigned)c.j);
                                         float* pp = (Pb + (n * (T * 10) * 132 + q * (10 * 132) + 64 + c.cb16)) + (__mul24(w, 132) + c.j);
                                         const f32x2 t0 = f32x2{v[0], v[1]} + f32x2{b4.x, b4.y}, t1 = f32x2{v[2], v[3]} + f32x2{b4.z, b4.w};
                                         const f32x2 m0 = t0 * slope6, m1 = t1 * slope6;
                                         const f32x2 r0 = f32x2{__builtin_amdgcn_fmed3f(t0[0], m0[0], pinf6), __builtin_amdgcn_fmed3f(t0[1], m0[1], pinf6)} + f32x2{e4.x, e4.y};
                                         const f32x2 r1 = f32x2{__builtin_amdgcn_fmed3f(t1[0], m1[0], pinf6), __builtin_amdgcn_fmed3f(t1[1], m1[1], pinf6)} + f32x2{e4.z, e4.w};
                                         lds_store4(lds_addr(pp), r0[0], r0[1], r1[0], r1[1]);
                                     });
        }
        if constexpr (MINW == 3 || (MINW >= 4 && T >= 5)) {
            tid = tid0;
            asm volatile("" : "+v"(tid));
            lane = tid & 63;
            wave = __builtin_amdgcn_readfirstlane(tid >> 6);
        }
        if constexpr (!EARLY2) rs_early(rc3, 2);
        if constexpr (!FUSE64) bsync();
        STAGE(11);
        lt_dump(6, RG + PL::L6_p + 64, 132, 64, 10);
        lt_inject(13, RG + PL::L6_p + 64, 132, 64, 10);
        if constexpr (LT) {
            if (P.lt_stage == 13) for (float& f : skip2) f = 0.f;
            if (P.lt_stage == 14) for (float& f : skip1) f = 0.f;
        }
        if constexpr (!EARLY2) mix_early(mc7, 7);
        resample_stage<64, 10, 12, T, NB, false, true, LOWO>(RG + PL::L6_p + 64, 132, RG + PL::UP3_out, 68, rc3, skip2, wave, lane);
        wearly(A7, MCD_LC(7));
        bsync();
        STAGE(12);
        lt_dump(13, RG + PL::UP3_out, 68, 64, 12);
        lt_inject(7, RG + PL::L7_in, 68, 64, 12);
        RsCoef<32, 12, 17, T, NB, false> rc4;
        LMix<9, T, NB> mc9;
        {
            constexpr int NT = PL::P12 / 16;
            constexpr int COLS = NB * T * 12;
            const LayerW lw = layer_w(wb, 8);
            float4 afr8[4];
            MixCoef<32, 12, T, NB> mc8w;
            layer_std<7, T, NB, LOWO>(wb, mc7, RG + PL::L7_in, RG + PL::L7_z, RG + PL::L7_out, EMB, wave, lane, prof, nohook,
                                [&] {
                                    load_afrags<4, 4>(reinterpret_cast<const float4*>(wptr<TSEL>(wb, lw.wp)), wave, lane, afr8, 0);
                                    if constexpr (EARLY2) mc8w.load(wptr<TSEL>(wb, lw.tq), wptr<TSEL>(wb, lw.am), wave, lane);
                                }, WEARLY ? &A7 : nullptr);
            STAGE(13);
            lt_dump(7, RG + PL::L7_out, 68, 64, 12);
            lt_inject(8, RG + PL::L8_in, 68, 64, 12);
            float* Pb = RG + PL::L8_p;
            if constexpr (!EARLY2) mc8w.load(wptr<TSEL>(wb, lw.tq), wptr<TSEL>(wb, lw.am), wave, lane);
            auto epi8 = [&](auto ti, int col, int c0, f32x4 acc, int col0, int) {
                constexpr int STEP = Tiling<4, NT>::NG * 16 * 68;
                constexpr bool FULL = TSEL && (decltype(ti)::value + 1) * Tiling<4, NT>::NG * 16 <= COLS;
                if (FULL || col < COLS) *reinterpret_cast<float4*>(Pb + __mul24(col0, 68) + c0 + decltype(ti)::value * STEP) = make_float4(acc[0], acc[1], acc[2], acc[3]);
            };
            gemm_tiles<4, NT, 4, 0, false, LOWO, LOWO, TSEL>(afr8, RG + PL::L8_in, 68, RG + PL::L8_in, 68, wave, lane, epi8, 0);
#pragma unroll
            for (int mi = 1; mi < Tiling<4, NT>::MW; ++mi) {
                load_afrags<4, 4>(reinterpret_cast<const float4*>(wptr<TSEL>(wb, lw.wp)), wave, lane, afr8, mi);
                gemm_tiles<4, NT, 4, 0, false, LOWO, LOWO, TSEL>(afr8, RG + PL::L8_in, 68, RG + PL::L8_in, 68, wave, lane, epi8, mi);
            }
            if constexpr (EARLY2) { rs_early(rc4, 3); mix_early(mc9, 9); }
            bsync();
            prof.mark(32 + 3 * 8 + 1);
            const float slope8 = lw.slope;
            const float pinf8 = prelu_bound(slope8);
            mix_stage<32, 12, T, NB, LOWO, true>(Pb, 68, mc8w, wptr<TSEL>(wb, lw.tq), wptr<TSEL>(wb, lw.am), wave, lane,
                                     [&](int n, int q, int w, ChIdx c) {
                                         const float* pp = (Pb + (n * (T * 12) * 68 + q * (12 * 68) + 32 + c.cb16)) + (__mul24(w, 68) + c.j);
                                         const float4 r = lds_load4(lds_addr(pp));
                                         return f32x4{r.x, r.y, r.z, r.w};
                                     },
                                     [&](int n, int q, int w, ChIdx c, f32x4 v) {
                                         const float4 b4 = lds_load4(lds_addr(BIA + 80 + c.cb16) + 4u * (unsigned)c.j);
                                         const float4 e4 = lds_load4(lds_addr(EMB + n * EMB_STRIDE + emb_off(8) + c.cb16) + 4u * (unsigned)c.j);
                                         float* pp = (Pb + (n * (T * 12) * 68 + q * (12 * 68) + 32 + c.cb16)) + (__mul24(w, 68) + c.j);
                                         const f32x2 t0 = f32x2{v[0], v[1]} + f32x2{b4.x, b4.y}, t1 = f32x2{v[2], v[3]} + f32x2{b4.z, b4.w};
                                         const f32x2 m0 = t0 * slope8, m1 = t1 * slope8;
                                         const f32x2 r0 = f32x2{__builtin_amdgcn_fmed3f(t0[0], m0[0], pinf8), __builtin_amdgcn_fmed3f(t0[1], m0[1], pinf8)} + f32x2{e4.x, e4.y};
                                         const f32x2 r1 = f32x2{__builtin_amdgcn_fmed3f(t1[0], m1[0], pinf8), __builtin_amdgcn_fmed3f(t1[1], m1[1], pinf8)} + f32x2{e4.z, e4.w};
                                         lds_store4(lds_addr(pp), r0[0], r0[1], r1[0], r1[1]);
                                     });
            if constexpr (!EARLY2) rs_early(rc4, 3);
            if constexpr (!SQ12) bsync();
            prof.mark(32 + 3 * 8);
            STAGE(14);
            lt_dump(8, RG + PL::L8_p + 32, 68, 32, 12);
            lt_inject(14, RG + PL::L8_p + 32, 68, 32, 12);
            if constexpr (!EARLY2) mix_early(mc9, 9);
            resample_stage<32, 12, 17, T, NB, false, true, LOWO, SQ12>(RG + PL::L8_p + 32, 68, RG + PL::UP2_out, 36, rc4, skip1, wave, lane);
        }
        wearly(A9, MCD_LC(9));
        bsync();
        STAGE(15);
        lt_dump(14, RG + PL::UP2_out, 36, 32, 17);
        lt_inject(9, RG + PL::L9_in, 36, 32, 17);
        {
            const LayerW lw = layer_w(wb, 10);
            MixCoef<16, 17, T, NB> mc10;
            EmbRow ef;
            auto ef_load = [&] { ef.template load<TSEL>(wb, tid); };
            layer_std<9, T, NB, LOWO>(wb, mc9, RG + PL::L9_in, RG + PL::L9_z, RG + PL::L9_out, EMB, wave, lane, prof,
                                [&] {
                                    mc10.load(wptr<TSEL>(wb, lw.tq), wptr<TSEL>(wb, lw.am), wave, lane);
                                    ef_load();
                                }, nohook, WEARLY ? &A9 : nullptr);
            STAGE(16);
            lt_dump(9, RG + PL::L9_out, 36, 32, 17);
            lt_inject(10, RG + PL::L10_in, 36, 32, 17);
            const float ca = srow[0], cb = srow[1], csg = srow[2];
            float* Pb = RG + PL::L10_p;
            {
                const int r = wave & 3;
                const cfloat* w4 = (const cfloat*)(wptr<TSEL>(wb, lw.wp) + r * 32);
                for (int cblk = wave >> 2; cblk * 64 < COLS17; cblk += NWAVES / 4) {
                    const int col = cblk * 64 + lane;
                    if (col < COLS17) {
                        const float* xp = RG + PL::L10_in + col * 36;
                        f32x2 acc2 = {0.f, 0.f};
#pragma unroll
                        for (int q = 0; q < 8; ++q) {
                            const float4 x = *reinterpret_cast<const float4*>(xp + 4 * q);
                            acc2 = f32x2{w4[4 * q + 0], w4[4 * q + 1]} * f32x2{x.x, x.y} + acc2;
                            acc2 = f32x2{w4[4 * q + 2], w4[4 * q + 3]} * f32x2{x.z, x.w} + acc2;
                        }
                        Pb[col * 20 + r] = acc2[0] + acc2[1];
                    }
                }
            }
            STAGE(18);
            emb_compute<NB>(ef, EXW, SEN, EMB, E10 + ((sidx - 1) & 1) * 16, tid);
            STAGE(19);
            bsync();
            STAGE(20);
            const float slope10 = lw.slope;
            const bool single = P.mode == 1, zadd = sidx > 1;
            const int e10_off = (sidx & 1) * 16;
            mix_stage<16, 17, T, NB, LOWO, true>(Pb, 20, mc10, wptr<TSEL>(wb, lw.tq), wptr<TSEL>(wb, lw.am), wave, lane,
                                     ZeroInit{},
                                     [&](int n, int t, int w, ChIdx c, auto val) {
                                         if constexpr (std::is_same_v<decltype(val), f32x4>) {
                                             if (c.j == 0) *reinterpret_cast<float2*>(ZO + ((n * T + t) * 17 + w) * C0) = make_float2(val[0], val[1]);
                                         } else {
                                             if (c.j < C0) ZO[((n * T + t) * 17 + w) * C0 + c.j] = val;
                                         }
                                     });
            bsync();
            constexpr int TAIL_IT = (COLS17 * C0 + NTHREADS - 1) / NTHREADS;
            float xn_t[TAIL_IT];
            int dst_t[TAIL_IT];
#pragma unroll
            for (int it = 0; it < TAIL_IT; ++it) {
                const int u = tid + it * NTHREADS;
                dst_t[it] = -1;
                xn_t[it] = 0.f;
                if (u < COLS17 * C0) {
                    const int c = u % C0, col = u / C0;
                    const int tt = TT[u];
                    const int n = (tt >> 4) & 3, t = (tt >> 6) & 15, v = tt >> 10;
                    const float x = XT[col * 4 + c];
                    const float l10 = prelu(ZO[u] + Pb[col * 20 + C0 + c] + BIA[64 + c], slope10) + E10[e10_off + n * 4 + c];
                    const float eps = l10 + x;
                    if constexpr (LT) {
                        const int b = win0 + n;
                        if (P.lt_stage == 10 && b < P.B) P.lt_out[(((size_t)b * C0 + c) * T + t) * 17 + v] = l10;
                    }
                    if (single) {
                        const int b = win0 + n;
                        if (b < P.B && P.eps_out) P.eps_out[(((size_t)b * C0 + c) * T + t) * 17 + v] = eps;
                    } else {
                        const int cbase = UPD[tt & 15];
                        if (cbase >= 0) {
                            const int colp = cbase + v;
                            const float z = zadd ? ZN[colp * C0 + c] : 0.f;
                            xn_t[it] = ca * (XT[colp * 4 + c] - cb * eps) + csg * z;
                            dst_t[it] = colp * 4 + c;
                        }
                    }
                }
            }
            if (P.upd_shift) bsync();
#pragma unroll
            for (int it = 0; it < TAIL_IT; ++it)
                if (dst_t[it] >= 0) XT[dst_t[it]] = xn_t[it];
            mc0.load(wptr<TSEL>(wb, tab_i(wb, F_TQ)), wptr<TSEL>(wb, tab_i(wb, F_AM)), wave, lane);
            wearly(A0, MCD_LC(0));
            STAGE(21);
            bsync();
            STAGE(17);
        }
    }
    if (P.mode == 1) break;

    float* RED = RG;
    const int per = CTV;
    {
        asm volatile("" : "+s"(Q));
        tid_s = tid0;
        asm volatile("" : "+v"(tid_s));
        DataView dv;
        dv.data = Q->dv.data; dv.base = Q->dv.base; dv.sc = Q->dv.sc; dv.st = Q->dv.st; dv.trans = Q->dv.trans; dv.aff = Q->dv.aff;
        const int seg_len = Q->seg_len, Bq = Q->B, Sq = Q->S, loss_fn = Q->loss_fn;
        float* pose_out = Q->pose_out;
        float* loss_out = Q->loss_out;
        const bool wmask = Q->win_mask != nullptr;
        for (int u = tid_s; u < NB * per; u += NTHREADS) {
            const int n = u / per, e = u % per;
            const int c = e / (Tx * 17), tx = (e / 17) % Tx, v = e % 17;
            const int solo = NB > 1 ? WM[9] : -1;
            const bool valid = win0 + n < Bq && (solo < 0 || n == solo);
            const int b = WM[4 + n];
            int tu = P.pos_of[tx];
            if (wmask) {
                const int fixed = WM[n];
                int cnt = 0;
                for (int t = 0; t < T; ++t)
                    if (!((fixed >> t) & 1)) { if (cnt == tx) tu = t; ++cnt; }
            }
            const float x0 = XT[((n * T + tu) * 17 + v) * 4 + c];
            const float gt = load_coord(dv, b, c, fm_src(P, tu), v, seg_len);
            const float d = fabsf(x0 - gt);
            float l;
            if (loss_fn == MCD_LOSS_SMOOTH_L1) l = d < 1.f ? 0.5f * d * d : d - 0.5f;
            else if (loss_fn == MCD_LOSS_L1) l = d;
            else l = d * d;
            RED[u] = l;
            if (valid && pose_out) pose_out[(size_t)(b * Sq + s) * per + e] = x0;
        }
        bsync();
        float* PART = RED + NB * per;
        if (tid_s < NB * 8) {
            const int n = tid_s >> 3, p8 = tid_s & 7;
            float sum = 0.f;
            for (int e = p8; e < per; e += 8) sum += RED[n * per + e];
            PART[tid_s] = sum;
        }
        bsync();
        if (tid_s < NB) {
            const int n = tid_s;
            float sum = 0.f;
#pragma unroll
            for (int k = 0; k < 8; ++k) sum += PART[n * 8 + k];
            const float l = sum / (float)per;
            const int solo = NB > 1 ? WM[9] : -1;
            if (solo < 0 || n == solo) {
                if (win0 + n < Bq && loss_out) loss_out[(size_t)(win0 + n) * Sq + s] = l;
                if (s < 64) LOSSB[n * 64 + s] = l;
                if (win0 + n < Bq && not_finite(l)) WM[8] = 1;
            }
        }
    }
    bsync();
    {
        const int div = WM[8], solo = NB > 1 ? WM[9] : -1;
        if (div) {
            for (int u = tid_s; u < PL::R + PL::XT; u += NTHREADS) smem[u] = 0.f;
            for (int u = tid_s; u < PL::ZN; u += NTHREADS) { ZN[u] = 0.f; ZO[u] = 0.f; }
        }
        if (NB > 1 && (div || solo >= 0)) {
            const int nxt = solo < 0 ? 0 : (solo + 1 < NB && win0 + solo + 1 < P.B ? solo + 1 : -1);
            if (nxt >= 0) s -= P.split;
            bsync();
            if (tid_s == 0) { WM[8] = 0; WM[9] = nxt; }
            bsync();
        } else if (div) {
            bsync();
            if (tid_s == 0) WM[8] = 0;
        }
    }
    }
#ifdef MCD_PROFILE
    __syncthreads();
    if (P.prof && tid0 == 0 && blockIdx.x < 6000) {
        unsigned hwid;
        asm volatile("s_getreg_b32 %0, hwreg(HW_REG_HW_ID)" : "=s"(hwid));
        unsigned xcc;
        asm volatile("s_getreg_b32 %0, hwreg(HW_REG_XCC_ID)" : "=s"(xcc));
        P.prof[4096 + 3 * blockIdx.x] = wg_t0;
        P.prof[4096 + 3 * blockIdx.x + 1] = __builtin_amdgcn_s_memrealtime();
        P.prof[4096 + 3 * blockIdx.x + 2] = ((unsigned long long)(xcc & 0xf) << 32) | hwid;
    }
    if (prof.on) {
        for (int i = 0; i < PROF_SLOTS; ++i) P.prof[i] += prof.acc[i];
        for (int i = 0; i < PL::PROFTR; ++i) P.prof[PROF_SLOTS + i] = prof.acc[PROF_SLOTS + i];
    }
#endif
    int te = tid0;
    asm volatile("" : "+v"(te));
    if constexpr (MINW >= 4) {
        if (P.mode == 0 && P.tune && blockIdx.x == 0 && te == 0) {
            P.tune[1] = (int)((unsigned)__builtin_amdgcn_s_memrealtime() - (unsigned)UPD[14]);
            P.tune[0] = (int)gridDim.x * 1009 + P.S * 31 + P.ns;
        }
    }
    if (P.mode == 0 && P.loss_agg && te < NB && win0 + te < P.B)
        P.loss_agg[win0 + te] = aggregate_losses(LOSSB + te * 64, P.S, P.aggr, P.aggr_q);
}

}
```

Before: 497,400.

## Precompute per-wave LDS stage addresses in a constexpr table for the 3x2 kernel

Adds a compile-time generated table of per-wave, per-stage LDS base addresses and coefficient offsets (StageRow) for the T=3, NB=2 scoring kernel. When it is selected, mix and resample stages read these bases from constant memory instead of computing unit-to-address arithmetic (div/mod by NQ, CB, multiplies) inside the kernel. The goal is to cut scalar and VALU address math and register pressure on the hot inner path, at the cost of extra scalar loads and a more complex template plumbing with static_assert coverage checks.

After: 506,000 (median of 6 runs). 1.7% higher.

```diff
diff --git a/mocodad_amd/csrc/mcd_device.hpp b/mocodad_amd/csrc/mcd_device.hpp
--- a/mocodad_amd/csrc/mcd_device.hpp
+++ b/mocodad_amd/csrc/mcd_device.hpp
@@ -25,6 +25,7 @@
 __device__ __forceinline__ gfloat* as_global(const float* p) { return (gfloat*)p; }
 typedef float __attribute__((address_space(3))) lds_float;
 typedef f32x4 __attribute__((address_space(3))) lds_f32x4;
+typedef f32x2 __attribute__((address_space(3))) lds_f32x2;
 __device__ __forceinline__ unsigned lds_addr(const float* p) { return (unsigned)(uintptr_t)p; }
 __device__ __forceinline__ float4 lds_load4(unsigned addr) {
     const f32x4 v = *(lds_f32x4*)(uintptr_t)addr;
@@ -245,7 +246,7 @@
     static constexpr int NR = (KS * T + 15) / 16;
     static constexpr bool SAMEQ = NQ == 3 && UNITS == 12 && NWAVES == 8;
     static_assert(T > 12 || PER == 1 || UNITS % NWAVES == 0 || SAMEQ, "mix units: a partial round of units (see MixCfg::QX)");
-    __device__ static __forceinline__ int unit_of(int wave, int round) {
+    __host__ __device__ static constexpr int unit_of(int wave, int round) {
         if constexpr (SAMEQ) {
             if (wave < 4) return (wave >> 1) + NQ * ((wave & 1) * 2 + round);
             return round == 0 ? 2 + NQ * (wave - 4) : -1;
@@ -262,6 +263,17 @@
     __device__ __forceinline__ void load(const float* tqd, const float* af, int wave, int lane) {
         load_unit(tqd, af, M::unit_of(wave, 0), lane);
     }
+    __device__ __forceinline__ void load_at(const float* tqd, const float* af, int lane) {
+        static_assert(M::QC == 1, "one output frame per unit");
+        gfloat* tqd_g = as_global(tqd);
+        gfloat* af_g = as_global(af);
+#pragma unroll
+        for (int r = 0; r < M::NR; ++r) tq[0][r] = tqd_g[r * 64 + lane];
+#pragma unroll
+        for (int mt = 0; mt < M::MT; ++mt)
+#pragma unroll
+            for (int ks = 0; ks < M::KS; ++ks) aop[0][mt][ks] = af_g[(mt * M::KS + ks) * 64 + lane];
+    }
     __device__ __forceinline__ void load_unit(const float* tqd, const float* af, int u, int lane) {
         gfloat* tqd_g = as_global(tqd);
         gfloat* af_g = as_global(af);
@@ -283,20 +295,44 @@
     int cb16, j;
     __device__ __forceinline__ operator int() const { return cb16 + j; }
 };
+struct StageRow { unsigned in_b, out_b, aux_b, aux2_b, tq_o, af_o, pad0, pad1; };
+typedef unsigned u32x4 __attribute__((ext_vector_type(4)));
+typedef unsigned u32x2 __attribute__((ext_vector_type(2)));
+typedef const u32x4 __attribute__((address_space(4))) cu32x4;
+typedef const u32x2 __attribute__((address_space(4))) cu32x2;
+__device__ __forceinline__ StageRow stage_row(const StageRow* tbw, int id, unsigned lds0) {
+    const u32x4 v = ((cu32x4*)tbw)[2 * id];
+    const u32x2 c = ((cu32x2*)tbw)[4 * id + 2];
+    return StageRow{v[0] + lds0, v[1] + lds0, v[2] + lds0, v[3] + lds0, c[0], c[1], 0u, 0u};
+}
+struct ChIdxRow {
+    int cb16, j;
+    unsigned ob, ab, ab2;
+    __device__ __forceinline__ operator int() const { return cb16 + j; }
+};
+template <bool ROWS>
+struct ChIdxOf {
+    __device__ static __forceinline__ auto make(int cb16, int jj, const StageRow* rows, int rnd) {
+        if constexpr (ROWS) return ChIdxRow{cb16, jj, rows[rnd].out_b, rows[rnd].aux_b, rows[rnd].aux2_b};
+        else return ChIdx{cb16, jj};
+    }
+};
 struct ZeroInit { __device__ __forceinline__ float operator()(int, int, int, int) const { return 0.f; } };
-template <int CIN, int V, int T, int NB, bool FORCE = false, bool SCORE = false, class Init, class Store>
+template <int CIN, int V, int T, int NB, bool FORCE = false, bool SCORE = false, bool ROWS = false, class Init, class Store>
 __device__ __forceinline__ void mix_stage(const float* __restrict__ in, int cs_in, const MixCoef<CIN, V, T, NB>& pre,
                                           const float* __restrict__ tqd, const float* __restrict__ af, int wave, int lane,
-                                          Init&& init, Store&& store) {
+                                          Init&& init, Store&& store, const StageRow* rows = nullptr) {
     using M = MixCfg<CIN, V, T, NB>;
     constexpr int KS = M::KS, KP = M::KP, MT = M::MT, CB = M::CB, QC = M::QC, NQ = M::NQ, PER = M::PER;
     constexpr bool XB32 = FORCE || SCORE;
     const int j = lane & 15, g = lane >> 4;
     const int voff_pair = 4 * (g & 1) + (g >> 1);
-    auto load_x = [&](int u, float (&x)[KS][T]) {
+    auto load_x = [&](int u, float (&x)[KS][T], int rnd) {
         const int rest = u / NQ;
         const int cb = rest % CB, n = rest / CB;
-        unsigned ua = lds_addr(in) + 4u * (unsigned)(n * (T * V) * cs_in + cb * 16);
+        unsigned ua;
+        if constexpr (ROWS) ua = rows[rnd].in_b;
+        else ua = lds_addr(in) + 4u * (unsigned)(n * (T * V) * cs_in + cb * 16);
         asm volatile("" : "+s"(ua));
         const lds_float* ub = (const lds_float*)(uintptr_t)ua;
         const lds_float* a_p = ub + (__mul24(voff_pair, cs_in) + j);
@@ -312,9 +348,11 @@
             }
         });
     };
-    auto unit = [&](const MixCoef<CIN, V, T, NB>& cur, int u, const float (&xs)[KS][T]) {
+    auto unit = [&](const MixCoef<CIN, V, T, NB>& cur, int u, const float (&xs)[KS][T], int rnd) {
         const int q0 = (u % NQ) * QC, rest = u / NQ;
         const int cb = rest % CB, n = rest / CB;
+        static_assert(!ROWS || (QC == 1 && !M::RAGGED), "stage-table rows: one output frame per unit");
+        auto chidx = [&](int jj) { return ChIdxOf<ROWS>::make(cb * 16, jj, rows, rnd); };
         constexpr bool J16 = V == 17;
         constexpr int MTM = J16 ? 1 : MT;
         constexpr bool ZINIT = std::is_same_v<std::decay_t<Init>, ZeroInit>;
@@ -329,7 +367,7 @@
                 if ((M::RAGGED && q0 + qi >= T) || ZINIT) {
                     acc[qi][mt] = f32x4{0.f, 0.f, 0.f, 0.f};
                 } else {
-                    acc[qi][mt] = init(n, q0 + qi, mt * 16 + j, ChIdx{cb * 16, 4 * g});
+                    acc[qi][mt] = init(n, q0 + qi, mt * 16 + j, chidx(4 * g));
                 }
         }
         static_for<KS>([&](auto si) {
@@ -356,7 +394,7 @@
             if (M::RAGGED && q0 + qi >= T) continue;
 #pragma unroll
             for (int mt = 0; mt < MTM; ++mt) {
-                if ((mt + 1) * 16 <= V || mt * 16 + j < V) store(n, q0 + qi, mt * 16 + j, ChIdx{cb * 16, 4 * g}, acc[qi][mt]);
+                if ((mt + 1) * 16 <= V || mt * 16 + j < V) store(n, q0 + qi, mt * 16 + j, chidx(4 * g), acc[qi][mt]);
             }
             if constexpr (J16) {
                 const unsigned u = __float_as_uint(part[qi]);
@@ -364,7 +402,7 @@
                 const unsigned v2 = __float_as_uint(__uint_as_float(h[0]) + __uint_as_float(h[1]));
                 const auto f = __builtin_amdgcn_permlane16_swap(v2, v2, false, false);
                 const float z16 = __uint_as_float(f[0]) + __uint_as_float(f[1]);
-                if (g == 0) store(n, q0 + qi, 16, ChIdx{cb * 16, j}, z16);
+                if (g == 0) store(n, q0 + qi, 16, chidx(j), z16);
             }
         }
     };
@@ -376,11 +414,11 @@
             const int u = ALLW ? wave + rnd * NWAVES : M::unit_of(wave, rnd);
             constexpr bool SURE = ALLW;
             float xs[KS][T];
-            load_x(SURE ? u : (u < 0 ? 0 : u), xs);
+            load_x(SURE ? u : (u < 0 ? 0 : u), xs, rnd);
             if constexpr (FORCE) __builtin_amdgcn_sched_barrier(0);
             MixCoef<CIN, V, T, NB> nxt;
             if constexpr (rnd + 1 < PER && !M::SAMEQ && NQ > 1) nxt.load_unit(tqd, af, M::unit_of(wave, rnd + 1), lane);
-            if (SURE || u >= 0) unit(cur, u, xs);
+            if (SURE || u >= 0) unit(cur, u, xs, rnd);
             if constexpr (rnd + 1 < PER && !M::SAMEQ && NQ > 1) cur = nxt;
         });
     }
@@ -428,10 +466,10 @@
     }
 };
 
-template <int C, int VIN, int VOUT, int T, int NB, bool CAPTURE, bool ADD, bool ILP = false, bool SQMAP = false, int NSK>
+template <int C, int VIN, int VOUT, int T, int NB, bool CAPTURE, bool ADD, bool ILP = false, bool SQMAP = false, bool ROWS = false, int NSK>
 __device__ __forceinline__ void resample_stage(const float* __restrict__ in, int cs_in, float* __restrict__ out, int cs_out,
                                                const RsCoef<C, VIN, VOUT, T, NB, CAPTURE>& rc,
-                                               float (&skip)[NSK], int wave, int lane) {
+                                               float (&skip)[NSK], int wave, int lane, const StageRow* rows = nullptr) {
     using RC = RsCfg<C, VIN, VOUT, T, NB, CAPTURE>;
     constexpr int KS = RC::KS, MT = RC::MT, CB = RC::CB, UNITS = RC::UNITS, PER = RC::PER, SK = RC::SK;
     static_assert(!(CAPTURE || ADD) || NSK == PER * SK, "skip register count");
@@ -459,17 +497,20 @@
         constexpr int i = decltype(pi)::value;
         int cb, nt;
         if (unit_at(i, cb, nt)) {
-            const float* ub = in + (nt * VIN * cs_in + cb * 16);
-            const float* a_main = ub + (__mul24(CAPTURE ? 4 * g : 4 * (g & 1) + (g >> 1), cs_in) + j);
-            const float* a_tail = CAPTURE ? ub + j : ub + (__mul24(g, cs_in) + j);
-            static_for<KS>([&](auto si) {
-                constexpr int ks = decltype(si)::value;
-                constexpr bool MAIN = CAPTURE ? ks < 4 : ks < KP;
-                constexpr int row0 = CAPTURE ? (ks < 4 ? ks : 16) : (ks < KP ? 8 * (ks >> 1) + 2 * (ks & 1) : 4 * KP);
-                const float xv = (MAIN ? a_main : a_tail)[row0 * cs_in];
-                if constexpr (CAPTURE) skip[i * SK + ks] = xv;
-                else xr[i][ks] = xv;
-            });
+            auto reads = [&](auto ub) {
+                const auto a_main = ub + (__mul24(CAPTURE ? 4 * g : 4 * (g & 1) + (g >> 1), cs_in) + j);
+                const auto a_tail = CAPTURE ? ub + j : ub + (__mul24(g, cs_in) + j);
+                static_for<KS>([&](auto si) {
+                    constexpr int ks = decltype(si)::value;
+                    constexpr bool MAIN = CAPTURE ? ks < 4 : ks < KP;
+                    constexpr int row0 = CAPTURE ? (ks < 4 ? ks : 16) : (ks < KP ? 8 * (ks >> 1) + 2 * (ks & 1) : 4 * KP);
+                    const float xv = (MAIN ? a_main : a_tail)[row0 * cs_in];
+                    if constexpr (CAPTURE) skip[i * SK + ks] = xv;
+                    else xr[i][ks] = xv;
+                });
+            };
+            if constexpr (ROWS) reads((const lds_float*)(uintptr_t)rows[i].in_b);
+            else reads(in + (nt * VIN * cs_in + cb * 16));
         }
     });
     constexpr bool J16 = VOUT == 17;
@@ -483,22 +524,25 @@
             for (int r = 0; r < 4; ++r) acc[0][r] += skip[i * SK + r];
             if constexpr (SK == 5 && !J16) acc[MT - 1][0] += skip[i * SK + 4];
         }
-        float* uo = out + (nt * VOUT * cs_out + cb * 16);
-        float* zo = uo + (__mul24(4 * g, cs_out) + j);
-#pragma unroll
-        for (int mt = 0; mt < MTM; ++mt)
-#pragma unroll
-            for (int r = 0; r < 4; ++r)
-                if (mt * 16 + 4 * g + r < VOUT) zo[(mt * 16 + r) * cs_out] = acc[mt][r];
-        if constexpr (J16) {
-            const unsigned pu = __float_as_uint(part);
-            const auto h = __builtin_amdgcn_permlane32_swap(pu, pu, false, false);
-            const unsigned v2 = __float_as_uint(__uint_as_float(h[0]) + __uint_as_float(h[1]));
-            const auto f = __builtin_amdgcn_permlane16_swap(v2, v2, false, false);
-            float z16 = __uint_as_float(f[0]) + __uint_as_float(f[1]) + bias[1][0];
-            if constexpr (ADD && SK == 5) z16 += skip[i * SK + 4];
-            if (g == 0) uo[16 * cs_out + j] = z16;
-        }
+        auto stores = [&](auto uo) {
+            const auto zo = uo + (__mul24(4 * g, cs_out) + j);
+#pragma unroll
+            for (int mt = 0; mt < MTM; ++mt)
+#pragma unroll
+                for (int r = 0; r < 4; ++r)
+                    if (mt * 16 + 4 * g + r < VOUT) zo[(mt * 16 + r) * cs_out] = acc[mt][r];
+            if constexpr (J16) {
+                const unsigned pu = __float_as_uint(part);
+                const auto h = __builtin_amdgcn_permlane32_swap(pu, pu, false, false);
+                const unsigned v2 = __float_as_uint(__uint_as_float(h[0]) + __uint_as_float(h[1]));
+                const auto f = __builtin_amdgcn_permlane16_swap(v2, v2, false, false);
+                float z16 = __uint_as_float(f[0]) + __uint_as_float(f[1]) + bias[1][0];
+                if constexpr (ADD && SK == 5) z16 += skip[i * SK + 4];
+                if (g == 0) uo[16 * cs_out + j] = z16;
+            }
+        };
+        if constexpr (ROWS) stores((lds_float*)(uintptr_t)rows[i].out_b);
+        else stores(out + (nt * VOUT * cs_out + cb * 16));
     };
     if constexpr (ILP) {
         f32x4 acc[PER][MTM];
@@ -773,7 +817,7 @@
                                               const float* __restrict__ in, float* __restrict__ z, float* __restrict__ out,
                                               const float* __restrict__ embl, int wave, int lane, Prof& prof, int prof_id,
                                               H1&& pre_gemm, H2&& pre_barrier,
-                                              const LayerAfr<(CIN / 16) * (RES ? 2 : 1)>* pre_afr = nullptr) {
+                                              const LayerAfr<(CIN / 16) * (RES ? 2 : 1)>* pre_afr = nullptr, const StageRow* rows = nullptr) {
     constexpr int MT = ceil16(COUT) / 16;
     constexpr int COLS = NB * T * V;
     constexpr int NT = ceil16(COLS) / 16;
@@ -784,6 +828,7 @@
     const int trs = 8 + 8 * ((prof_id - 32) / 3);
     prof.trace(trs + 0);
     constexpr bool TSEL = SLOTSEL && HASEMB && NB == 2 && T == 3;
+    constexpr bool ROWS = TSEL && MixCfg<CIN, V, T, NB>::QC == 1;
     const float* bias = wptr<TSEL>(wb, lw.bias);
     float4 bcur;
     if (pre_afr != nullptr) {
@@ -794,13 +839,19 @@
         load_afrags<MT, KQ1 + KQ2>(reinterpret_cast<const float4*>(wptr<TSEL>(wb, lw.wp)), wave, lane, afr);
         bcur = load_global4(bias + (wave % MT) * 16 + 4 * (lane >> 4));
     }
-    mix_stage<CIN, V, T, NB, FORCE, HASEMB>(in, CSX, mc, wptr<TSEL>(wb, lw.tq), wptr<TSEL>(wb, lw.am), wave, lane,
+    mix_stage<CIN, V, T, NB, FORCE, HASEMB, ROWS>(in, CSX, mc, wptr<TSEL>(wb, lw.tq), wptr<TSEL>(wb, lw.am), wave, lane,
                              ZeroInit{},
-                             [&](int n, int q, int w, ChIdx c, auto v) {
+                             [&](int n, int q, int w, auto c, auto v) {
+                                 if constexpr (ROWS) {
+                                     const unsigned za = c.ob + 4u * (unsigned)(__mul24(w, CSI) + c.j);
+                                     if constexpr (std::is_same_v<decltype(v), f32x4>) lds_store4(za, v[0], v[1], v[2], v[3]);
+                                     else *(lds_float*)(uintptr_t)za = v;
+                                 } else {
                                  float* zp = (z + (n * (T * V) * CSI + q * (V * CSI) + c.cb16)) + (__mul24(w, CSI) + c.j);
                                  if constexpr (std::is_same_v<decltype(v), f32x4>) lds_store4(lds_addr(zp), v[0], v[1], v[2], v[3]);
                                  else *zp = v;
-                             });
+                                 }
+                             }, rows);
     prof.trace(trs + 1);
     pre_gemm();
     bsync();
@@ -916,10 +967,10 @@
 template <int L, int T, int NB, bool FORCE = false, int CSX = cs_of(layer_desc(L).cin), class H1, class H2>
 __device__ __forceinline__ void layer_std(const float* wb, const LMix<L, T, NB>& mc, const float* in, float* z, float* out,
                                           const float* emb, int wave, int lane, Prof& prof, H1&& pre_gemm, H2&& pre_barrier,
-                                          const LAfr<L>* pre_afr = nullptr) {
+                                          const LAfr<L>* pre_afr = nullptr, const StageRow* rows = nullptr) {
     constexpr LDesc D = layer_desc(L);
     layer_generic<D.cin, D.cout, D.V, D.res != 0, true, T, NB, FORCE, CSX, true>(wb, layer_w(wb, L), mc, in, z, out, emb + emb_off(L), wave, lane,
-                                                               prof, 32 + 3 * L, pre_gemm, pre_barrier, pre_afr);
+                                                               prof, 32 + 3 * L, pre_gemm, pre_barrier, pre_afr, rows);
 }
 
 struct EmbRow {
@@ -1010,6 +1061,8 @@
     static constexpr int TOTAL = R + XT + EMB + EAUX + ZN + WM + BIA + UPD + ZO + TT + CE + LOSS + EXW + PROF;
     static_assert((size_t)TOTAL * 4 <= 160 * 1024, "LDS plan: more than 160 KB");
     static constexpr size_t BYTES = (size_t)TOTAL * 4;
-};
-
-}
+    static constexpr int O_XT = R, O_EMB = O_XT + XT, O_E10 = O_EMB + EMB, O_ZN = O_E10 + EAUX, O_WM = O_ZN + ZN, O_BIA = O_WM + WM,
+                         O_UPD = O_BIA + BIA, O_ZO = O_UPD + UPD;
+};
+
+}
diff --git a/mocodad_amd/csrc/mcd_score_kernel.hpp b/mocodad_amd/csrc/mcd_score_kernel.hpp
--- a/mocodad_amd/csrc/mcd_score_kernel.hpp
+++ b/mocodad_amd/csrc/mcd_score_kernel.hpp
@@ -1,6 +1,7 @@
 #pragma once
 #include "mcd_device.hpp"
 #include "mcd_encode_kernel.hpp"
+#include "mcd_stage_table.hpp"
 
 namespace mcd {
 
@@ -11,15 +12,15 @@
     constexpr int COLS17 = NB * TV17;
     extern __shared__ __attribute__((aligned(16))) float smem[];
     float* const RG = smem;
-    float* const XT = RG + PL::R;
-    float* const EMB = XT + PL::XT;
-    float* const E10 = EMB + PL::EMB;
+    float* const XT = smem + PL::O_XT;
+    float* const EMB = smem + PL::O_EMB;
+    float* const E10 = smem + PL::O_E10;
     float* const SEN = E10 + 32;
-    float* const ZN = E10 + PL::EAUX;
-    int* const WM = reinterpret_cast<int*>(ZN + PL::ZN);
-    float* const BIA = reinterpret_cast<float*>(WM + PL::WM);
-    int* const UPD = reinterpret_cast<int*>(BIA + PL::BIA);
-    float* const ZO = reinterpret_cast<float*>(UPD + PL::UPD);
+    float* const ZN = smem + PL::O_ZN;
+    int* const WM = reinterpret_cast<int*>(smem + PL::O_WM);
+    float* const BIA = smem + PL::O_BIA;
+    int* const UPD = reinterpret_cast<int*>(smem + PL::O_UPD);
+    float* const ZO = smem + PL::O_ZO;
 
     const int tid0 = threadIdx.x;
     int tid = tid0;
@@ -149,6 +150,23 @@
     float skip2[RS2::PER * RS2::SK];
     constexpr bool LOWO = MINW <= (NWAVES == 12 ? 3 : 2);
     constexpr bool TSEL = T == 3 && NB == 2;
+    const unsigned lds0 = (unsigned)(uintptr_t)(lds_float*)smem;
+    const StageRow* tbw = nullptr;
+    auto stage_rows_of = [&](int wv) {
+        if constexpr (TSEL) {
+            static_assert(stage_tab_checked<T, NB>());
+            const StageRow* tb = &StageTab<T, NB>::tab.r[0][0];
+            asm volatile("" : "+s"(tb));
+            tbw = tb + wv * srow::NROWS;
+        }
+    };
+    auto srows = [&](auto& r, int id) {
+        if constexpr (TSEL) {
+#pragma unroll
+            for (int k = 0; k < (int)std::extent_v<std::remove_reference_t<decltype(r)>>; ++k) r[k] = stage_row(tbw, id + k, lds0);
+        }
+    };
+    StageRow r0[1], r1[1], r2[2], rdn1[2], r3[2], r8[2], rup2[2], r9[2], r10[1];
 
     const int i_first = P.mode == 1 ? P.step_single : P.ns - 1;
     const int i_last = P.mode == 1 ? P.step_single : 1;
@@ -211,6 +229,8 @@
     constexpr bool WEARLY = T <= 4;
     LAfr<0> A0;
     if constexpr (WEARLY) load_lafr<0>(A0, P.wbuf, wave, lane);
+    stage_rows_of(wave);
+    srows(r0, srow::L0);
     for (int sidx = i_first; sidx >= i_last; --sidx) {
         const float* srow = P.step_table + sidx * (4 + EDIM);
         const float* wb = P.wbuf;
@@ -219,6 +239,7 @@
         asm volatile("" : "+v"(tid));
         lane = tid & 63;
         wave = __builtin_amdgcn_readfirstlane(tid >> 6);
+        stage_rows_of(wave);
         if constexpr (MINW >= 4) {
             const int sh = UPD[15];
             if (sh > 0) {
@@ -267,6 +288,12 @@
 #endif
         auto mixload = [&](auto& mc, int l) { mc.load(wptr<TSEL>(wb, tab_i(wb, l * F_STRIDE + F_TQ)), wptr<TSEL>(wb, tab_i(wb, l * F_STRIDE + F_AM)), wave, lane); };
         auto rsload = [&](auto& rc, int r) { rc.load(wptr<TSEL>(wb, tab_i(wb, TAB_RSW + r)), wptr<TSEL>(wb, tab_i(wb, TAB_RSB + r)), lane); };
+        auto wptrb = [&](unsigned bytes) { return reinterpret_cast<const float*>(reinterpret_cast<const char*>(wb) + bytes); };
+        auto mixrow_at = [&](auto& mc, int tq, int am, const StageRow& r) { mc.load_at(wptrb(4u * (unsigned)tq + r.tq_o), wptrb(4u * (unsigned)am + r.af_o), lane); };
+        auto mixrows = [&](auto& mc, int l, auto& r, int id) {
+            if constexpr (TSEL) { srows(r, id); mixrow_at(mc, tab_i(wb, l * F_STRIDE + F_TQ), tab_i(wb, l * F_STRIDE + F_AM), r[0]); }
+            else mixload(mc, l);
+        };
         auto mix_early = mixload;
         auto rs_early = rsload;
         NoHook nohook;
@@ -276,27 +303,27 @@
         auto wearly = [&](auto& A, auto lc) { if constexpr (WEARLY) load_lafr<decltype(lc)::value, TSEL>(A, wb, wave, lane); };
 #define MCD_LC(l) std::integral_constant<int, l>{}
         layer_std<0, T, NB, LOWO, 4>(wb, mc0, XT, RG + PL::L0_z, RG + PL::L0_out, EMB, wave, lane, prof,
-                            [&] { mix_early(mc1, 1); }, [&] { wearly(A1, MCD_LC(1)); }, WEARLY ? &A0 : nullptr);
+                            [&] { mixrows(mc1, 1, r1, srow::L1); }, [&] { wearly(A1, MCD_LC(1)); }, WEARLY ? &A0 : nullptr, r0);
         STAGE(2);
         lt_dump(0, RG + PL::L0_out, 20, 16, 17);
         lt_inject(1, RG + PL::L1_in, 20, 16, 17);
         LMix<2, T, NB> mc2;
         silu_row(sidx > 0 ? sidx - 1 : 0, tid - NZ_T0);
         layer_std<1, T, NB, LOWO>(wb, mc1, RG + PL::L1_in, RG + PL::L1_z, RG + PL::L1_out, EMB, wave, lane, prof,
-                            [&] { mix_early(mc2, 2); }, [&] { wearly(A2, MCD_LC(2)); }, WEARLY ? &A1 : nullptr);
+                            [&] { mixrows(mc2, 2, r2, srow::L2); }, [&] { wearly(A2, MCD_LC(2)); }, WEARLY ? &A1 : nullptr, r1);
         STAGE(3);
         lt_dump(1, RG + PL::L1_out, 36, 32, 17);
         lt_inject(2, RG + PL::L2_in, 36, 32, 17);
         RsCoef<32, 17, 12, T, NB, true> rc1;
         LMix<3, T, NB> mc3;
+        constexpr bool SQ12 = !LT && MixCfg<32, 12, T, NB>::SAMEQ;
         layer_std<2, T, NB, LOWO>(wb, mc2, RG + PL::L2_in, RG + PL::L2_z, RG + PL::L2_out, EMB, wave, lane, prof,
-                            [&] { rs_early(rc1, 0); }, [&] { if constexpr (EARLY2) mix_early(mc3, 3); }, WEARLY ? &A2 : nullptr);
+                            [&] { rs_early(rc1, 0); if constexpr (SQ12) srows(rdn1, srow::DN1); }, [&] { if constexpr (EARLY2) mixrows(mc3, 3, r3, srow::L3); }, WEARLY ? &A2 : nullptr, r2);
         STAGE(4);
         lt_dump(2, RG + PL::L2_out, 36, 32, 17);
         lt_inject(11, RG + PL::L2_out, 36, 32, 17);
-        if constexpr (!EARLY2) mix_early(mc3, 3);
-        constexpr bool SQ12 = !LT && MixCfg<32, 12, T, NB>::SAMEQ;
-        resample_stage<32, 17, 12, T, NB, true, false, LOWO, SQ12>(RG + PL::L2_out, 36, RG + PL::DN1_out, 36, rc1, skip1, wave, lane);
+        if constexpr (!EARLY2) mixrows(mc3, 3, r3, srow::L3);
+        resample_stage<32, 17, 12, T, NB, true, false, LOWO, SQ12, TSEL && SQ12>(RG + PL::L2_out, 36, RG + PL::DN1_out, 36, rc1, skip1, wave, lane, rdn1);
         wearly(A3, MCD_LC(3));
         bsync();
         STAGE(5);
@@ -304,7 +331,7 @@
         lt_inject(3, RG + PL::L3_in, 36, 32, 12);
         LMix<4, T, NB> mc4;
         layer_std<3, T, NB, LOWO>(wb, mc3, RG + PL::L3_in, RG + PL::L3_z, RG + PL::L3_out, EMB, wave, lane, prof,
-                            [&] { mix_early(mc4, 4); }, [&] { wearly(A4, MCD_LC(4)); }, WEARLY ? &A3 : nullptr);
+                            [&] { mix_early(mc4, 4); }, [&] { wearly(A4, MCD_LC(4)); }, WEARLY ? &A3 : nullptr, r3);
         STAGE(6);
         lt_dump(3, RG + PL::L3_out, 68, 64, 12);
         lt_inject(4, RG + PL::L4_in, 68, 64, 12);
@@ -413,7 +440,11 @@
             lt_dump(7, RG + PL::L7_out, 68, 64, 12);
             lt_inject(8, RG + PL::L8_in, 68, 64, 12);
             float* Pb = RG + PL::L8_p;
-            if constexpr (!EARLY2) mc8w.load(wptr<TSEL>(wb, lw.tq), wptr<TSEL>(wb, lw.am), wave, lane);
+            srows(r8, srow::L8);
+            if constexpr (!EARLY2) {
+                if constexpr (TSEL) mixrow_at(mc8w, lw.tq, lw.am, r8[0]);
+                else mc8w.load(wptr<TSEL>(wb, lw.tq), wptr<TSEL>(wb, lw.am), wave, lane);
+            }
             auto epi8 = [&](auto ti, int col, int c0, f32x4 acc, int col0, int) {
                 constexpr int STEP = Tiling<4, NT>::NG * 16 * 68;
                 constexpr bool FULL = TSEL && (decltype(ti)::value + 1) * Tiling<4, NT>::NG * 16 <= COLS;
@@ -425,18 +456,32 @@
                 load_afrags<4, 4>(reinterpret_cast<const float4*>(wptr<TSEL>(wb, lw.wp)), wave, lane, afr8, mi);
                 gemm_tiles<4, NT, 4, 0, false, LOWO, LOWO, TSEL>(afr8, RG + PL::L8_in, 68, RG + PL::L8_in, 68, wave, lane, epi8, mi);
             }
-            if constexpr (EARLY2) { rs_early(rc4, 3); mix_early(mc9, 9); }
+            if constexpr (EARLY2) { rs_early(rc4, 3); if constexpr (SQ12) srows(rup2, srow::UP2); mixrows(mc9, 9, r9, srow::L9); }
             bsync();
             prof.mark(32 + 3 * 8 + 1);
             const float slope8 = lw.slope;
             const float pinf8 = prelu_bound(slope8);
-            mix_stage<32, 12, T, NB, LOWO, true>(Pb, 68, mc8w, wptr<TSEL>(wb, lw.tq), wptr<TSEL>(wb, lw.am), wave, lane,
-                                     [&](int n, int q, int w, ChIdx c) {
+            mix_stage<32, 12, T, NB, LOWO, true, TSEL>(Pb, 68, mc8w, wptr<TSEL>(wb, lw.tq), wptr<TSEL>(wb, lw.am), wave, lane,
+                                     [&](int n, int q, int w, auto c) {
+                                         if constexpr (TSEL) {
+                                             const float4 r = lds_load4(c.ob + 4u * (unsigned)(__mul24(w, 68) + c.j));
+                                             return f32x4{r.x, r.y, r.z, r.w};
+                                         } else {
                                          const float* pp = (Pb + (n * (T * 12) * 68 + q * (12 * 68) + 32 + c.cb16)) + (__mul24(w, 68) + c.j);
                                          const float4 r = lds_load4(lds_addr(pp));
                                          return f32x4{r.x, r.y, r.z, r.w};
+                                         }
                                      },
-                                     [&](int n, int q, int w, ChIdx c, f32x4 v) {
+                                     [&](int n, int q, int w, auto c, f32x4 v) {
+                                         if constexpr (TSEL) {
+                                             const float4 b4 = lds_load4(c.ab2 + 4u * (unsigned)c.j);
+                                             const float4 e4 = lds_load4(c.ab + 4u * (unsigned)c.j);
+                                             const f32x2 t0 = f32x2{v[0], v[1]} + f32x2{b4.x, b4.y}, t1 = f32x2{v[2], v[3]} + f32x2{b4.z, b4.w};
+                                             const f32x2 m0 = t0 * slope8, m1 = t1 * slope8;
+                                             const f32x2 r0 = f32x2{__builtin_amdgcn_fmed3f(t0[0], m0[0], pinf8), __builtin_amdgcn_fmed3f(t0[1], m0[1], pinf8)} + f32x2{e4.x, e4.y};
+                                             const f32x2 r1 = f32x2{__builtin_amdgcn_fmed3f(t1[0], m1[0], pinf8), __builtin_amdgcn_fmed3f(t1[1], m1[1], pinf8)} + f32x2{e4.z, e4.w};
+                                             lds_store4(c.ob + 4u * (unsigned)(__mul24(w, 68) + c.j), r0[0], r0[1], r1[0], r1[1]);
+                                         } else {
                                          const float4 b4 = lds_load4(lds_addr(BIA + 80 + c.cb16) + 4u * (unsigned)c.j);
                                          const float4 e4 = lds_load4(lds_addr(EMB + n * EMB_STRIDE + emb_off(8) + c.cb16) + 4u * (unsigned)c.j);
                                          float* pp = (Pb + (n * (T * 12) * 68 + q * (12 * 68) + 32 + c.cb16)) + (__mul24(w, 68) + c.j);
@@ -445,15 +490,16 @@
                                          const f32x2 r0 = f32x2{__builtin_amdgcn_fmed3f(t0[0], m0[0], pinf8), __builtin_amdgcn_fmed3f(t0[1], m0[1], pinf8)} + f32x2{e4.x, e4.y};
                                          const f32x2 r1 = f32x2{__builtin_amdgcn_fmed3f(t1[0], m1[0], pinf8), __builtin_amdgcn_fmed3f(t1[1], m1[1], pinf8)} + f32x2{e4.z, e4.w};
                                          lds_store4(lds_addr(pp), r0[0], r0[1], r1[0], r1[1]);
-                                     });
-            if constexpr (!EARLY2) rs_early(rc4, 3);
+                                         }
+                                     }, r8);
+            if constexpr (!EARLY2) { rs_early(rc4, 3); if constexpr (SQ12) srows(rup2, srow::UP2); }
             if constexpr (!SQ12) bsync();
             prof.mark(32 + 3 * 8);
             STAGE(14);
             lt_dump(8, RG + PL::L8_p + 32, 68, 32, 12);
             lt_inject(14, RG + PL::L8_p + 32, 68, 32, 12);
-            if constexpr (!EARLY2) mix_early(mc9, 9);
-            resample_stage<32, 12, 17, T, NB, false, true, LOWO, SQ12>(RG + PL::L8_p + 32, 68, RG + PL::UP2_out, 36, rc4, skip1, wave, lane);
+            if constexpr (!EARLY2) mixrows(mc9, 9, r9, srow::L9);
+            resample_stage<32, 12, 17, T, NB, false, true, LOWO, SQ12, TSEL && SQ12>(RG + PL::L8_p + 32, 68, RG + PL::UP2_out, 36, rc4, skip1, wave, lane, rup2);
         }
         wearly(A9, MCD_LC(9));
         bsync();
@@ -467,9 +513,11 @@
             auto ef_load = [&] { ef.template load<TSEL>(wb, tid); };
             layer_std<9, T, NB, LOWO>(wb, mc9, RG + PL::L9_in, RG + PL::L9_z, RG + PL::L9_out, EMB, wave, lane, prof,
                                 [&] {
-                                    mc10.load(wptr<TSEL>(wb, lw.tq), wptr<TSEL>(wb, lw.am), wave, lane);
+                                    srows(r10, srow::L10);
+                                    if constexpr (TSEL) mixrow_at(mc10, lw.tq, lw.am, r10[0]);
+                                    else mc10.load(wptr<TSEL>(wb, lw.tq), wptr<TSEL>(wb, lw.am), wave, lane);
                                     ef_load();
-                                }, nohook, WEARLY ? &A9 : nullptr);
+                                }, nohook, WEARLY ? &A9 : nullptr, r9);
             STAGE(16);
             lt_dump(9, RG + PL::L9_out, 36, 32, 17);
             lt_inject(10, RG + PL::L10_in, 36, 32, 17);
@@ -501,15 +549,23 @@
             const float slope10 = lw.slope;
             const bool single = P.mode == 1, zadd = sidx > 1;
             const int e10_off = (sidx & 1) * 16;
-            mix_stage<16, 17, T, NB, LOWO, true>(Pb, 20, mc10, wptr<TSEL>(wb, lw.tq), wptr<TSEL>(wb, lw.am), wave, lane,
+            mix_stage<16, 17, T, NB, LOWO, true, TSEL>(Pb, 20, mc10, wptr<TSEL>(wb, lw.tq), wptr<TSEL>(wb, lw.am), wave, lane,
                                      ZeroInit{},
-                                     [&](int n, int t, int w, ChIdx c, auto val) {
+                                     [&](int n, int t, int w, auto c, auto val) {
+                                         if constexpr (TSEL) {
+                                             lds_float* zo = (lds_float*)(uintptr_t)c.ob;
+                                             if constexpr (std::is_same_v<decltype(val), f32x4>) {
+                                                 if (c.j == 0) *(lds_f32x2*)(zo + w * C0) = f32x2{val[0], val[1]};
+                                             } else {
+                                                 if (c.j < C0) zo[w * C0 + c.j] = val;
+                                             }
+                                         } else
                                          if constexpr (std::is_same_v<decltype(val), f32x4>) {
                                              if (c.j == 0) *reinterpret_cast<float2*>(ZO + ((n * T + t) * 17 + w) * C0) = make_float2(val[0], val[1]);
                                          } else {
                                              if (c.j < C0) ZO[((n * T + t) * 17 + w) * C0 + c.j] = val;
                                          }
-                                     });
+                                     }, r10);
             bsync();
             constexpr int TAIL_IT = (COLS17 * C0 + NTHREADS - 1) / NTHREADS;
             float xn_t[TAIL_IT];
@@ -548,7 +604,9 @@
 #pragma unroll
             for (int it = 0; it < TAIL_IT; ++it)
                 if (dst_t[it] >= 0) XT[dst_t[it]] = xn_t[it];
-            mc0.load(wptr<TSEL>(wb, tab_i(wb, F_TQ)), wptr<TSEL>(wb, tab_i(wb, F_AM)), wave, lane);
+            srows(r0, srow::L0);
+            if constexpr (TSEL) mixrow_at(mc0, tab_i(wb, F_TQ), tab_i(wb, F_AM), r0[0]);
+            else mc0.load(wptr<TSEL>(wb, tab_i(wb, F_TQ)), wptr<TSEL>(wb, tab_i(wb, F_AM)), wave, lane);
             wearly(A0, MCD_LC(0));
             STAGE(21);
             bsync();
diff --git a/mocodad_amd/csrc/mcd_stage_table.hpp b/mocodad_amd/csrc/mcd_stage_table.hpp
--- /dev/null
+++ b/mocodad_amd/csrc/mcd_stage_table.hpp
@@ -0,0 +1,124 @@
+#pragma once
+#include "mcd_device.hpp"
+
+namespace mcd {
+
+namespace srow { enum { L0 = 0, L1 = 1, L2 = 2, DN1 = 4, L3 = 6, L8 = 8, UP2 = 10, L9 = 12, L10 = 14, NROWS = 16 }; }
+
+template <int T, int NB>
+struct StageTabGen {
+    static_assert(T == 3 && NB == 2 && NWAVES == 8, "the stage table is generated for the 3-frame x 2-chain kernel of 8 waves");
+    using PL = Plan<T, NB>;
+    using M16 = MixCfg<16, 17, T, NB>;
+    using M17 = MixCfg<32, 17, T, NB>;
+    using M12 = MixCfg<32, 12, T, NB>;
+    static_assert(M16::QC == 1 && M16::UNITS == 6 && M16::PER == 1 && M17::SAMEQ && M12::SAMEQ && M17::PER == 2 && M12::PER == 2, "unit maps the rows are generated for");
+    enum { L0 = srow::L0, L1 = srow::L1, L2 = srow::L2, DN1 = srow::DN1, L3 = srow::L3, L8 = srow::L8, UP2 = srow::UP2, L9 = srow::L9, L10 = srow::L10, NROWS = srow::NROWS };
+    struct Tab { StageRow r[NWAVES][NROWS]; };
+
+    struct Unit { int n, cb, q; };
+    template <class M>
+    static constexpr Unit unit(int wave, int round) {
+        const int um = M::unit_of(wave, round);
+        const int u = um < 0 ? 0 : um;
+        const int rest = u / M::NQ;
+        return Unit{rest / M::CB, rest % M::CB, (u % M::NQ) * M::QC};
+    }
+    template <class M>
+    static constexpr StageRow mix_row(int wave, int round, int V, int in, int cs_in, int out, int cs_out, int aux = 0, int aux2 = 0) {
+        const Unit u = unit<M>(wave, round);
+        return StageRow{4u * (unsigned)(in + u.n * (T * V) * cs_in + u.cb * 16),
+                        4u * (unsigned)(out + u.n * (T * V) * cs_out + u.q * (V * cs_out) + u.cb * 16),
+                        4u * (unsigned)(aux + u.n * EMB_STRIDE + u.cb * 16), 4u * (unsigned)(aux2 + u.cb * 16),
+                        4u * (unsigned)(u.q * M::NR * 64), 4u * (unsigned)(u.q * M::MT * M::KS * 64), 0u, 0u};
+    }
+    static constexpr StageRow rs_row(int wave, int slot, int in, int vin, int cs_in, int out, int vout, int cs_out) {
+        const Unit u = unit<M12>(wave, slot);
+        const int nt = u.n * T + u.q;
+        return StageRow{4u * (unsigned)(in + nt * vin * cs_in + u.cb * 16), 4u * (unsigned)(out + nt * vout * cs_out + u.cb * 16), 0u, 0u, 0u, 0u, 0u, 0u};
+    }
+    static constexpr Tab make() {
+        Tab t{};
+        for (int w = 0; w < NWAVES; ++w) {
+            StageRow* r = t.r[w];
+            r[L0] = mix_row<M16>(w, 0, 17, PL::O_XT, 4, PL::L0_z, 20);
+            r[L1] = mix_row<M16>(w, 0, 17, PL::L1_in, 20, PL::L1_z, 20);
+            r[L10] = mix_row<M16>(w, 0, 17, PL::L10_p, 20, PL::O_ZO, 2);
+            for (int k = 0; k < 2; ++k) {
+                r[L2 + k] = mix_row<M17>(w, k, 17, PL::L2_in, 36, PL::L2_z, 36);
+                r[L9 + k] = mix_row<M17>(w, k, 17, PL::L9_in, 36, PL::L9_z, 36);
+                r[L3 + k] = mix_row<M12>(w, k, 12, PL::L3_in, 36, PL::L3_z, 36);
+                r[L8 + k] = mix_row<M12>(w, k, 12, PL::L8_p, 68, PL::L8_p + 32, 68, PL::O_EMB + emb_off(8), PL::O_BIA + 80);
+                r[DN1 + k] = rs_row(w, k, PL::L2_out, 17, 36, PL::DN1_out, 12, 36);
+                r[UP2 + k] = rs_row(w, k, PL::L8_p + 32, 12, 68, PL::UP2_out, 17, 36);
+            }
+        }
+        return t;
+    }
+};
+template <int T, int NB>
+struct StageTab : StageTabGen<T, NB> {
+    using G = StageTabGen<T, NB>;
+    using typename G::Tab;
+    using typename G::Unit;
+    using typename G::PL;
+    using typename G::M12;
+    using typename G::M17;
+    static constexpr Tab tab = G::make();
+
+    static constexpr bool sameq_closed_form() {
+        for (int w = 0; w < NWAVES; ++w)
+            for (int k = 0; k < 2; ++k) {
+                if (w >= 4 && k == 1) { if (M12::unit_of(w, k) >= 0 || M17::unit_of(w, k) >= 0) return false; continue; }
+                const Unit a = G::template unit<M12>(w, k), b = G::template unit<M17>(w, k);
+                const Unit c = w < 4 ? Unit{w & 1, k, w >> 1} : Unit{(w - 4) >> 1, w & 1, 2};
+                if (a.n != c.n || a.cb != c.cb || a.q != c.q || b.n != c.n || b.cb != c.cb || b.q != c.q) return false;
+            }
+        return true;
+    }
+    static constexpr bool covers(int row, int rounds, int ncb, unsigned in0, unsigned in_n, unsigned in_q, unsigned out0, unsigned out_n, unsigned out_q, unsigned tq_q = 0u, unsigned af_q = 0u) {
+        for (int n = 0; n < NB; ++n)
+            for (int cb = 0; cb < ncb; ++cb)
+                for (int q = 0; q < T; ++q) {
+                    int hits = 0;
+                    for (int w = 0; w < NWAVES; ++w)
+                        for (int k = 0; k < rounds; ++k) {
+                            if (rounds == 1 ? w >= 6 : (k == 1 && w >= 4)) continue;
+                            const StageRow& r = tab.r[w][row + k];
+                            if (r.in_b == in0 + n * in_n + q * in_q + cb * 64u && r.out_b == out0 + n * out_n + q * out_q + cb * 64u &&
+                                (tq_q == 0u || (r.tq_o == q * tq_q && r.af_o == q * af_q))) ++hits;
+                        }
+                    if (hits != 1) return false;
+                }
+        return true;
+    }
+    static constexpr bool in_plan() {
+        for (int w = 0; w < NWAVES; ++w)
+            for (int i = 0; i < G::NROWS; ++i) {
+                const StageRow& r = tab.r[w][i];
+                if (r.in_b % 16 || r.out_b % 8 || r.aux_b % 16 || r.aux2_b % 16) return false;
+                if (r.in_b >= PL::BYTES || r.out_b >= PL::BYTES || r.aux_b >= PL::BYTES || r.aux2_b >= PL::BYTES) return false;
+            }
+        return true;
+    }
+};
+template <int T, int NB>
+constexpr bool stage_tab_checked() {
+    using S = StageTab<T, NB>;
+    using PL = Plan<T, NB>;
+    constexpr unsigned TV17 = T * 17, TV12 = T * 12;
+    static_assert(S::sameq_closed_form(), "SAMEQ unit map: not the closed form the rows were checked against");
+    static_assert(S::in_plan(), "a stage-table row points outside the LDS plan or is misaligned");
+    static_assert(S::covers(S::L0, 1, 1, 4u * PL::O_XT, 4u * TV17 * 4, 0u, 4u * PL::L0_z, 4u * TV17 * 20, 4u * 17 * 20, 256u, 4u * 2 * 5 * 64), "layer 0 rows");
+    static_assert(S::covers(S::L1, 1, 1, 4u * PL::L1_in, 4u * TV17 * 20, 0u, 4u * PL::L1_z, 4u * TV17 * 20, 4u * 17 * 20, 256u, 4u * 2 * 5 * 64), "layer 1 rows");
+    static_assert(S::covers(S::L10, 1, 1, 4u * PL::L10_p, 4u * TV17 * 20, 0u, 4u * PL::O_ZO, 4u * TV17 * 2, 4u * 17 * 2, 256u, 4u * 2 * 5 * 64), "layer 10 rows");
+    static_assert(S::covers(S::L2, 2, 2, 4u * PL::L2_in, 4u * TV17 * 36, 0u, 4u * PL::L2_z, 4u * TV17 * 36, 4u * 17 * 36, 256u, 4u * 2 * 5 * 64), "layer 2 rows");
+    static_assert(S::covers(S::L9, 2, 2, 4u * PL::L9_in, 4u * TV17 * 36, 0u, 4u * PL::L9_z, 4u * TV17 * 36, 4u * 17 * 36, 256u, 4u * 2 * 5 * 64), "layer 9 rows");
+    static_assert(S::covers(S::L3, 2, 2, 4u * PL::L3_in, 4u * TV12 * 36, 0u, 4u * PL::L3_z, 4u * TV12 * 36, 4u * 12 * 36, 256u, 4u * 1 * 3 * 64), "layer 3 rows");
+    static_assert(S::covers(S::L8, 2, 2, 4u * PL::L8_p, 4u * TV12 * 68, 0u, 4u * (PL::L8_p + 32), 4u * TV12 * 68, 4u * 12 * 68, 256u, 4u * 1 * 3 * 64), "layer 8 rows");
+    static_assert(S::covers(S::DN1, 2, 2, 4u * PL::L2_out, 4u * TV17 * 36, 4u * 17 * 36, 4u * PL::DN1_out, 4u * TV12 * 36, 4u * 12 * 36), "down1 rows");
+    static_assert(S::covers(S::UP2, 2, 2, 4u * (PL::L8_p + 32), 4u * TV12 * 68, 4u * 12 * 68, 4u * PL::UP2_out, 4u * TV17 * 36, 4u * 17 * 36), "up2 rows");
+    return true;
+}
+
+}
```
